# MyrtleSoftware/myrtle-vision

Measured on AMD Instinct MI355X. Metric: images/sec (train fwd+bwd) ViT-B/16 224^2 bf16, higher is better.
Workload: dtype bf16

## Files before the change

### include/myrtle_vision_hip.h

```cpp
#ifndef MYRTLE_VISION_HIP_H
#define MYRTLE_VISION_HIP_H

#include <stddef.h>
#include <stdint.h>

#ifdef __cplusplus
extern "C" {
#endif

typedef void* mv_stream_t;

enum { MV_F32 = 0, MV_BF16 = 1, MV_I8 = 2 , MV_F16 = 3  };

enum {
  MV_OK = 0,
  MV_ERR_SHAPE = -1,
  MV_ERR_ALIGN = -2,
  MV_ERR_LAUNCH = -3,
  MV_ERR_UNSUPPORTED = -4,
  MV_ERR_WORKSPACE = -5
};

enum {
  MV_EPI_NONE = 0,
  MV_EPI_GELU = 1,
  MV_EPI_RESIDUAL = 2,
  MV_EPI_DGELU = 3,
  MV_EPI_GELU_GRAD = 5,
  MV_EPI_MUL = 6,
  MV_EPI_GELU_Q8 = 7,
  MV_EPI_GELU_GRAD8 = 8,
  MV_EPI_MUL8 = 9,
  MV_EPI_SPLIT_DGELU = 10,
  MV_EPI_SPLIT_GELU = 11,
  MV_EPI_EMBED = 4
};

int mv_version(void);
const char* mv_error_string(int code);
size_t mv_gemm_tn_workspace_bytes(int M, int N, int Kc);
int mv_gemm_force_variant(int nt_variant, int tn_variant);
size_t mv_layernorm_bwd_workspace_bytes(int rows, int dim);

int mv_layernorm_fwd(const float* x, long ldx, const float* gamma, const float* beta, void* y, int y_dtype,
                     float* mean, float* rstd, int rows, int dim, float eps, mv_stream_t stream);
int mv_layernorm_fwd_split(const float* x, long ldx, const float* gamma, const float* beta, void* y_split, int nseg, float* mean,
                           float* rstd, int rows, int dim, float eps, mv_stream_t stream);
int mv_layernorm_bwd(const void* dy, int dy_dtype, const float* x, long ldx, const float* gamma,
                     const float* mean, const float* rstd, const float* dx_add, float* dx, long lddx,
                     float* dgamma, float* dbeta, int accumulate, float* workspace, size_t workspace_bytes,
                     int rows, int dim, void* dx_bf16, float* dx_colsum, mv_stream_t stream);
int mv_layernorm_bwd_split(const void* dy, int dy_dtype, const float* x, long ldx, const float* gamma, const float* mean,
                           const float* rstd, const float* dx_add, float* dx, long lddx, float* dgamma, float* dbeta, int accumulate,
                           float* workspace, size_t workspace_bytes, int rows, int dim, void* dx_split, int nseg, float* dx_colsum,
                           mv_stream_t stream);

int mv_gemm_nt_bf16(const void* A, int lda, const void* B, int ldb, void* C, int ldc, int c_dtype, int M, int N,
                    int K, const float* bias, int epilogue, const void* aux, int ld_aux, int aux_i, void* out2,
                    int ld_out2, mv_stream_t stream);
int mv_gemm_nt_bf16_scaled(const void* A, int lda, const void* B, int ldb, void* C, int ldc, int c_dtype, int M, int N,
                           int K, float alpha, const float* bias, int epilogue, const void* aux, int ld_aux, int aux_i,
                           void* out2, int ld_out2, mv_stream_t stream);
int mv_gemm_tn_bf16(const void* A, int lda, const void* B, int ldb, float* C, int ldc, int M, int N, int Kc,
                    int accumulate, float* colsum, float* workspace, size_t workspace_bytes, mv_stream_t stream);

int mv_gemm_f32(const float* A, long sa_m, long sa_k, long sa_b1, long sa_b2, const float* B, long sb_k, long sb_n,
                long sb_b1, long sb_b2, float* C, long sc_m, long sc_n, long sc_b1, long sc_b2, int M, int N, int K,
                int nb1, int nb2, float alpha, int accumulate, const float* bias, int epilogue, const float* aux,
                long ld_aux, int aux_i, float* out2, long ld_out2, mv_stream_t stream);
int mv_sum_slabs(const float* slabs, long stride, int S, float* out, long n, int accumulate, mv_stream_t stream);
int mv_sum_slabs_add(const float* slabs, long stride, int S, const float* add, float* out, long n, mv_stream_t stream);
int mv_gemm_f32_force_fma(int on);

int mv_attention_fwd(const void* qkv, void* out, float* lse, int B, int N, int H, float scale, mv_stream_t stream);
int mv_attention_bwd(const void* qkv, const void* out, const void* dout, const float* lse, void* dqkv, float* colsum,
                     int B, int N, int H, float scale, mv_stream_t stream);
int mv_attention_fwd_f16(const void* qkv16, float* out, float* lse, int B, int N, int H, float scale, mv_stream_t stream);
int mv_attention_bwd_prep_f16(const float* dout, const float* out, void* dout16, float* delta, float* gscale, int B, int N, int H,
                              mv_stream_t stream);
int mv_attention_bwd_f16(const void* qkv16, const void* dout16, const float* delta, const float* lse, const float* gscale,
                         void* dqkv, int nseg, float* colsum, int B, int N, int H, float scale, mv_stream_t stream);
int mv_attention_bwd_force(int variant);
int mv_attention_fwd_force(int variant);
int mv_attention_fwd_f32(const float* qkv, float* out, int B, int N, int H, float scale, mv_stream_t stream);

int mv_softmax_fwd(const float* x, float* y, long rows, int cols, float scale, mv_stream_t stream);
int mv_softmax_bwd(const float* y, const float* dy, float* dx, long rows, int cols, float scale, mv_stream_t stream);

int mv_patchify(const float* img, void* out, int out_dtype, int B, int C, int H, int W, int p, mv_stream_t stream);
int mv_embed_cls(const float* cls, const float* pos, float* x, int B, int T, int D, mv_stream_t stream);
int mv_embed_bwd(const float* dx, float* dpos, float* dcls, int accumulate, int B, int T, int D, mv_stream_t stream);
int mv_embed_bwd_gather(const float* dx, void* dy, int dy_dtype, float* dpos, float* dcls, int B, int T, int D,
                        mv_stream_t stream);
int mv_gather_patch_rows(const float* src, void* dst, int dst_dtype, int B, int T, int D, mv_stream_t stream);

int mv_cast(const void* src, int src_dtype, void* dst, int dst_dtype, long n, mv_stream_t stream);
int mv_split3_bf16(const float* x, long ldx, void* out, long ldo, long seg, long rows, int cols, int role,
                   mv_stream_t stream);
size_t mv_split3_ex_workspace_bytes(long rows, int cols);
int mv_split3_bf16_ex(const float* x, long ldx, const float* h, long ldh, int op, void* out, long rows, int cols,
                      float* colsum, float* workspace, size_t workspace_bytes, mv_stream_t stream);
int mv_gemm_nt_bf16_ksplit(const void* A, int lda, const void* B, int ldb, float* slabs, int M, int N, int K, int splits,
                           const float* bias, mv_stream_t stream);
int mv_gemm_tn_bf16_x6(const void* A6, const void* B6, float* C, int ldc, int M, int N, int rows, float* workspace,
                       size_t workspace_bytes, mv_stream_t stream);
int mv_split2_bf16(const float* x, long ldx, void* out, long ldo, long seg, long rows, int cols, int role,
                   mv_stream_t stream);
int mv_split2_bf16_ex(const float* x, long ldx, const float* h, long ldh, int op, void* out, long rows, int cols,
                      float* colsum, float* workspace, size_t workspace_bytes, mv_stream_t stream);
int mv_weight_split(const float* w, void* fwd, void* dx, int R, int C, int nseg, mv_stream_t stream);
int mv_split_f8c(const float* x, long ldx, void* out, long ldo_bytes, long rows, int cols, int role, int exp_hi, mv_stream_t stream);
int mv_gemm_nt_f8c(const void* A, long lda_bytes, const void* B, long ldb_bytes, void* C, int ldc, int c_dtype, int M, int N, int K,
                   int scale_exp, const float* bias, int epilogue, const void* aux, int ld_aux, mv_stream_t stream);
int mv_gemm_tn_bf16_x3(const void* A3, const void* B3, float* C, int ldc, int M, int N, int rows, float* workspace,
                       size_t workspace_bytes, mv_stream_t stream);
int mv_weight_prep(const float* w, void* w_bf16, int ldw, void* wt_bf16, int ldt, int R, int C, mv_stream_t stream);
typedef struct mv_weight_prep_item {
  const float* w;
  void* w_bf16;
  void* wt_bf16;
  int ldw, ldt, R, C;
  int tiles_x, first_block;
} mv_weight_prep_item;
int mv_weight_prep_batch(const mv_weight_prep_item* items_device, int count, int total_blocks, mv_stream_t stream);
int mv_colsum(const void* x, int x_dtype, long ld, float* out, int accumulate, long rows, int cols, float* workspace,
              size_t workspace_bytes, mv_stream_t stream);
int mv_gelu_fwd(const void* x, void* y, int dtype, long n, mv_stream_t stream);
int mv_gelu_bwd(const void* x, const void* dy, void* dx, int dtype, long n, mv_stream_t stream);
int mv_add_f32(const float* a, const float* b, float* out, long n, mv_stream_t stream);

int mv_quant_float(const float* x, float* y, long n, int exp_bits, int man_bits, mv_stream_t stream);
int mv_quant_fixed(const float* x, float* y, long n, int wl, int fl, int clamp, int symmetric, mv_stream_t stream);
int mv_quant_affine(const float* x, float* y, long n, float scale, int zero_point, int qmin, int qmax,
                    mv_stream_t stream);
int mv_quant_affine_codes(const void* x, int x_dtype, void* codes, long rows, int cols, int ld, float scale, int zero_point,
                          int qmin, int qmax, int pre_op, mv_stream_t stream);
int mv_quant_float_f16(const float* x, void* y, long n, mv_stream_t stream);
int mv_gemm_nt_f16(const void* A, int lda, const void* B, int ldb, void* C, int ldc, int M, int N, int K, const float* bias,
                   int epilogue, const void* aux, int ld_aux, void* out2, int ld_out2, mv_stream_t stream);
int mv_quant_affine_i8(const void* x, int x_dtype, void* codes, long rows, int cols, int ld, float scale, int zero_point,
                       int pre_op, mv_stream_t stream);
int mv_gemm_nt_i8(const void* A, int lda, const void* B, int ldb, void* C, int ldc, int c_dtype, int M, int N, int K,
                  float alpha, const float* bias, const int* icorr, int epilogue, const void* aux, int ld_aux,
                  float q_scale, int q_zero_point, mv_stream_t stream);
int mv_attention_fwd_f32_lse(const float* qkv, float* out, float* lse, int B, int N, int H, float scale, mv_stream_t stream);
// ... 51 lines not shown
```

### myrtle-vision_amd/csrc/gemm_bf16.hip

```cpp
#include "mv_common.h"

#include <atomic>
#include <type_traits>

namespace {

constexpr int BM = 128, BN = 128, BK = 64;
constexpr int STAGE_BYTES = (BM + BN) * BK * 2;
constexpr int SMEM_BYTES = 2 * STAGE_BYTES;

__device__ __forceinline__ int sw128(int row, int ch) { return row * 128 + ((ch ^ (((row >> 1) & 3) << 1)) << 4); }
__device__ __forceinline__ int sw256(int row, int ch) {
  return row * 256 + ((ch ^ (((row & 3) << 2) | ((row >> 2) & 3))) << 4);
}

__device__ __forceinline__ int xcd_remap(int bid, int nwg) {
  const int q = nwg >> 3, r = nwg & 7, xcd = bid & 7, idx = bid >> 3;
  return (xcd < r ? xcd * (q + 1) : r * (q + 1) + (xcd - r) * q) + idx;
}

struct EpiArgs {
  float alpha;
  const float* bias;
  const void* aux;
  int ld_aux;
  int aux_i;
  void* out2;
  int ld_out2;
  const int* icorr;
  float q_inv, q_zp;
  int ks_tiles, ks_len;
  long ks_slab;
  int band;
  int f8_tiles16, f8_scale;
};

__device__ __forceinline__ void st16(void* p, u32x4 v) { *reinterpret_cast<u32x4*>(p) = v; }

template <typename CT>
__device__ __forceinline__ void store4(CT* p, const float v[4], bool vec, int nvalid) {
  if (vec) {
    if constexpr (sizeof(CT) == 4) {
      *reinterpret_cast<float4*>(p) = make_float4(v[0], v[1], v[2], v[3]);
    } else {
      typedef CT ct4 __attribute__((ext_vector_type(4)));
      const ct4 o = {(CT)v[0], (CT)v[1], (CT)v[2], (CT)v[3]};
      *reinterpret_cast<ct4*>(p) = o;
    }
  } else {
#pragma unroll
    for (int r = 0; r < 4; ++r)
      if (r < nvalid) p[r] = (CT)v[r];
  }
}

__device__ __forceinline__ void nt_colsum_flush(float (&cs)[4][4], float* __restrict__ partial, int ld, int row_block, int nb,
                                                int N, int lane) {
#pragma unroll
  for (int j = 0; j < 4; ++j)
#pragma unroll
    for (int r = 0; r < 4; ++r) {
      float v = cs[j][r];
      v += __shfl_xor(v, 1, 64);
      v += __shfl_xor(v, 2, 64);
      v += __shfl_xor(v, 4, 64);
      v += __shfl_xor(v, 8, 64);
      cs[j][r] = v;
    }
  if ((lane & 15) == 0) {
#pragma unroll
    for (int j = 0; j < 4; ++j)
#pragma unroll
      for (int r = 0; r < 4; ++r) {
        const int n = nb + j * 16 + r;
        if (n < N) partial[(long)row_block * ld + n] = cs[j][r];
      }
  }
}

__device__ __forceinline__ float erf_fast(float u, float& e) { return mv_erf_fast(u, e); }
__device__ __forceinline__ float gelu_fast(float x) {
  float e;
  return 0.5f * x * (1.0f + erf_fast(x * 0.70710678118654752440f, e));
}
__device__ __forceinline__ void gelu_both_fast(float x, float& gl, float& dg) {
  float e;
  const float cdf = 0.5f * (1.0f + erf_fast(x * 0.70710678118654752440f, e));
  gl = x * cdf;
  dg = fmaf(x * 0.39894228040143267794f, e, cdf);
}
constexpr bool epi_is_gelu(int e) { return e == MV_EPI_GELU || e == MV_EPI_GELU_GRAD || e == MV_EPI_GELU_GRAD8; }
constexpr bool epi_is_dgelu(int e) { return e == MV_EPI_DGELU || e == MV_EPI_MUL || e == MV_EPI_MUL8; }
constexpr bool epi_is_gelugrad(int e) { return e == MV_EPI_GELU_GRAD || e == MV_EPI_GELU_GRAD8; }
constexpr bool epi_is_split(int e) { return e == MV_EPI_SPLIT_DGELU || e == MV_EPI_SPLIT_GELU; }
__device__ __forceinline__ void store_pieces4(bf16_t* o, const float (&v)[4], int nseg, long seg) {
  bf16x4 p[3];
#pragma unroll
  for (int e = 0; e < 4; ++e) {
    const bf16_t p0 = (bf16_t)v[e];
    const float r1 = v[e] - (float)p0;
    const bf16_t p1 = (bf16_t)r1;
    p[0][e] = p0;
    p[1][e] = p1;
    p[2][e] = (bf16_t)(r1 - (float)p1);
  }
  *reinterpret_cast<bf16x4*>(o) = p[0];
  *reinterpret_cast<bf16x4*>(o + seg) = p[0];
  *reinterpret_cast<bf16x4*>(o + 2 * seg) = p[1];
  if (nseg == 6) {
    *reinterpret_cast<bf16x4*>(o + 3 * seg) = p[0];
    *reinterpret_cast<bf16x4*>(o + 4 * seg) = p[1];
    *reinterpret_cast<bf16x4*>(o + 5 * seg) = p[2];
  }
}
constexpr float GQ_STEP = 0.005f, GQ_INV = 200.0f, GQ_ZERO = 26.0f;
__device__ __forceinline__ unsigned gq_code(float g) {
  return (unsigned)__builtin_amdgcn_fmed3f(fmaf(g, GQ_INV, GQ_ZERO + 0.5f), 0.f, 255.f);
}
__device__ __forceinline__ unsigned gq_pack4(const float (&g)[4]) {
  return gq_code(g[0]) | (gq_code(g[1]) << 8) | (gq_code(g[2]) << 16) | (gq_code(g[3]) << 24);
}
__device__ __forceinline__ float gq_value(float code) { return (code - GQ_ZERO) * GQ_STEP; }
__device__ __forceinline__ float gq_decode(unsigned w, int k) { return gq_value((float)((w >> (8 * k)) & 255u)); }
__device__ __forceinline__ float dgelu_fast(float x) {
  float e;
  const float cdf = 0.5f * (1.0f + erf_fast(x * 0.70710678118654752440f, e));
  return fmaf(x * 0.39894228040143267794f, e, cdf);
}

template <typename CT = bf16_t>
__device__ __forceinline__ u32x4 pair_swap_bf16(const float (&va)[4], const float (&vb)[4]) {
  typedef CT ct4 __attribute__((ext_vector_type(4)));
  const ct4 pa = {(CT)va[0], (CT)va[1], (CT)va[2], (CT)va[3]};
  const ct4 pb = {(CT)vb[0], (CT)vb[1], (CT)vb[2], (CT)vb[3]};
  typedef unsigned u32x2_t __attribute__((ext_vector_type(2)));
  const u32x2_t a = __builtin_bit_cast(u32x2_t, pa), b = __builtin_bit_cast(u32x2_t, pb);
  const u32x2_t r0 = __builtin_amdgcn_permlane16_swap(a[0], b[0], false, false);
  const u32x2_t r1 = __builtin_amdgcn_permlane16_swap(a[1], b[1], false, false);
  return (u32x4){r0[0], r1[0], r0[1], r1[1]};
}

template <int EPI>
struct EpiPre {
  float4 ax[EPI == MV_EPI_RESIDUAL ? 4 : 1][EPI == MV_EPI_RESIDUAL ? 4 : 1];
  u32x4 xq[EPI == MV_EPI_MUL8 ? 4 : 1];
};
template <int EPI>
__device__ __forceinline__ void nt_epi_prefetch(EpiPre<EPI>& P, int m0, int n0, int wm, int wn, int lane, const EpiArgs& ep) {
  const int mb = m0 + wm * 64 + (lane & 15), nb = n0 + wn * 64 + 4 * (lane >> 4);
  if constexpr (EPI == MV_EPI_RESIDUAL) {
#pragma unroll
    for (int i = 0; i < 4; ++i)
#pragma unroll
      for (int j = 0; j < 4; ++j)
        P.ax[i][j] = *reinterpret_cast<const float4*>(reinterpret_cast<const float*>(ep.aux) + (long)(mb + i * 16) * ep.ld_aux + nb + j * 16);
  } else if constexpr (EPI == MV_EPI_MUL8) {
    const unsigned char* a8 = reinterpret_cast<const unsigned char*>(ep.aux);
#pragma unroll
    for (int i = 0; i < 4; ++i)
      P.xq[i] = *reinterpret_cast<const u32x4*>(a8 + (long)(mb + i * 16) * ep.ld_aux + n0 + wn * 64 + 16 * (lane >> 4));
  }
}
template <int EPI>
__device__ __forceinline__ bool nt_epi_prefetch_ok(int M, int N, int m0, int n0, int ldc, const EpiArgs& ep) {
  const bool interior = (m0 + BM <= M) && (n0 + BN <= N) && ((ldc & 3) == 0) && ((ep.ld_aux & 3) == 0) &&
                        ((ep.ld_out2 & 3) == 0) && ((reinterpret_cast<uintptr_t>(ep.bias) & 15) == 0);
  if constexpr (EPI == MV_EPI_MUL8)
    return interior && (ep.ld_aux & 15) == 0 && (reinterpret_cast<uintptr_t>(ep.aux) & 15) == 0;
  return interior && EPI == MV_EPI_RESIDUAL;
}

template <int EPI, typename CT, bool PRE = false>
__device__ __forceinline__ void nt_epilogue(f32x4 (&acc)[4][4], CT* __restrict__ C, int ldc, int M, int N, int m0, int n0,
                                            int wm, int wn, int lane, const EpiArgs& ep, const float* bias_lds = nullptr,
                                            const EpiPre<EPI>& pre = EpiPre<EPI>{}) {
  const bool interior = (m0 + BM <= M) && (n0 + BN <= N) && ((ldc & 3) == 0) && ((ep.ld_aux & 3) == 0) &&
                        ((ep.ld_out2 & 3) == 0) && ((reinterpret_cast<uintptr_t>(ep.bias) & 15) == 0);
  if (interior) {
    const int mb = m0 + wm * 64 + (lane & 15), nb = n0 + wn * 64 + 4 * (lane >> 4);
    float4 bv[4];
#pragma unroll
    for (int j = 0; j < 4; ++j)
      bv[j] = bias_lds ? *reinterpret_cast<const float4*>(bias_lds + wn * 64 + 4 * (lane >> 4) + j * 16)
              : (!epi_is_dgelu(EPI) && ep.bias) ? *reinterpret_cast<const float4*>(ep.bias + nb + j * 16)
                                                : make_float4(0.f, 0.f, 0.f, 0.f);
    long crow[4];
    int prow[4];
#pragma unroll
    for (int i = 0; i < 4; ++i) {
      const int m = mb + i * 16;
      crow[i] = m;
      prow[i] = 0;
      if constexpr (EPI == MV_EPI_EMBED) {
        const int img = m / ep.aux_i;
        prow[i] = 1 + (m - img * ep.aux_i);
        crow[i] = (long)img * (ep.aux_i + 1) + prow[i];
      }
    }
    if constexpr (EPI == MV_EPI_GELU_Q8) {
      const bool wide = (ldc & 15) == 0 && (reinterpret_cast<uintptr_t>(C) & 15) == 0;
#pragma unroll
      for (int i = 0; i < 4; ++i) {
        unsigned w[4];
#pragma unroll
        for (int j = 0; j < 4; ++j) {
          const float v0 = fmaf(acc[i][j][0], ep.alpha, bv[j].x), v1 = fmaf(acc[i][j][1], ep.alpha, bv[j].y);
          const float v2 = fmaf(acc[i][j][2], ep.alpha, bv[j].z), v3 = fmaf(acc[i][j][3], ep.alpha, bv[j].w);
          w[j] = affine_i8_pack4<1>(v0, v1, v2, v3, ep.q_inv, ep.q_zp);
        }
        char* crow8 = reinterpret_cast<char*>(C) + (long)(mb + i * 16) * ldc;
        if (wide) {
          typedef unsigned u32x2_t __attribute__((ext_vector_type(2)));
          const u32x2_t s01 = __builtin_amdgcn_permlane16_swap(w[0], w[1], false, false);
          const u32x2_t s23 = __builtin_amdgcn_permlane16_swap(w[2], w[3], false, false);
          const u32x2_t t02 = __builtin_amdgcn_permlane32_swap(s01[0], s23[0], false, false);
          const u32x2_t t13 = __builtin_amdgcn_permlane32_swap(s01[1], s23[1], false, false);
          st16(crow8 + n0 + wn * 64 + 16 * (lane >> 4), (u32x4){t02[0], t13[0], t02[1], t13[1]});
        } else {
#pragma unroll
          for (int j = 0; j < 4; ++j) *reinterpret_cast<unsigned*>(crow8 + nb + j * 16) = w[j];
        }
      }
      return;
    }
    float4 ax[4][4];
    if constexpr (EPI == MV_EPI_RESIDUAL || EPI == MV_EPI_EMBED || EPI == MV_EPI_SPLIT_DGELU) {
#pragma unroll
      for (int i = 0; i < 4; ++i)
#pragma unroll
        for (int j = 0; j < 4; ++j) {
          if constexpr (EPI == MV_EPI_RESIDUAL && PRE) {
            ax[i][j] = pre.ax[i][j];
            continue;
          }
          const long arow = (EPI == MV_EPI_EMBED) ? prow[i] : (mb + i * 16);
          ax[i][j] = *reinterpret_cast<const float4*>(reinterpret_cast<const float*>(ep.aux) + arow * ep.ld_aux + nb + j * 16);
        }
    }
    bf16x4 hx[4][4];
    unsigned hq[4][4];
    if constexpr (EPI == MV_EPI_MUL8) {
      const unsigned char* a8 = reinterpret_cast<const unsigned char*>(ep.aux);
      if ((ep.ld_aux & 15) == 0 && (reinterpret_cast<uintptr_t>(a8) & 15) == 0) {
        typedef unsigned u32x2_t __attribute__((ext_vector_type(2)));
        u32x4 x[4];
#pragma unroll
        for (int i = 0; i < 4; ++i)
          x[i] = PRE ? pre.xq[i]
                     : *reinterpret_cast<const u32x4*>(a8 + (long)(mb + i * 16) * ep.ld_aux + n0 + wn * 64 + 16 * (lane >> 4));
#pragma unroll
        for (int i = 0; i < 4; ++i) {
          const u32x2_t s01 = __builtin_amdgcn_permlane16_swap(x[i][0], x[i][1], false, false);
          const u32x2_t s23 = __builtin_amdgcn_permlane16_swap(x[i][2], x[i][3], false, false);
          const u32x2_t t02 = __builtin_amdgcn_permlane32_swap(s01[0], s23[0], false, false);
          const u32x2_t t13 = __builtin_amdgcn_permlane32_swap(s01[1], s23[1], false, false);
// ... 42 lines not shown
                    gelu_both_fast(v[q][r], gl, dg);
                    hpre[q][r] = dg;
                    v[q][r] = gl;
                  } else {
                    hpre[q][r] = v[q][r];
                    v[q][r] = gelu_fast(v[q][r]);
                  }
                }
              } else if constexpr (epi_is_dgelu(EPI)) {
#pragma unroll
                for (int r = 0; r < 4; ++r)
                  v[q][r] *= (EPI == MV_EPI_MUL8) ? gq_decode(hq[i][j], r)
                             : (EPI == MV_EPI_MUL) ? (float)hx[i][j][r] : dgelu_fast((float)hx[i][j][r]);
                cs[j][0] += v[q][0]; cs[j][1] += v[q][1]; cs[j][2] += v[q][2]; cs[j][3] += v[q][3];
              }
            }
            if constexpr (EPI == MV_EPI_GELU_GRAD8) {
              gw[2 * jp] = gq_pack4(hpre[0]);
              gw[2 * jp + 1] = gq_pack4(hpre[1]);
            } else if constexpr (epi_is_gelu(EPI)) {
              if (ep.out2)
                st16(reinterpret_cast<bf16_t*>(ep.out2) + (long)(mb + i * 16) * ep.ld_out2 + nw + 32 * jp,
                     pair_swap_bf16(hpre[0], hpre[1]));
            }
            st16(C + crow[i] * ldc + nw + 32 * jp, pair_swap_bf16<CT>(v[0], v[1]));
          }
          if constexpr (EPI == MV_EPI_GELU_GRAD8) {
            if (ep.out2) {
              typedef unsigned u32x2_t __attribute__((ext_vector_type(2)));
              const u32x2_t s01 = __builtin_amdgcn_permlane16_swap(gw[0], gw[1], false, false);
              const u32x2_t s23 = __builtin_amdgcn_permlane16_swap(gw[2], gw[3], false, false);
              const u32x2_t t02 = __builtin_amdgcn_permlane32_swap(s01[0], s23[0], false, false);
              const u32x2_t t13 = __builtin_amdgcn_permlane32_swap(s01[1], s23[1], false, false);
              st16(reinterpret_cast<unsigned char*>(ep.out2) + (long)(mb + i * 16) * ep.ld_out2 + n0 + wn * 64 + 16 * (lane >> 4),
                   (u32x4){t02[0], t13[0], t02[1], t13[1]});
            }
          }
        }
        if constexpr (epi_is_dgelu(EPI)) {
          if (ep.out2) nt_colsum_flush(cs, reinterpret_cast<float*>(ep.out2), ep.ld_out2, (m0 + wm * 64) >> 6, nb, N, lane);
        }
        return;
      }
    }
#pragma unroll
    for (int i = 0; i < 4; ++i)
#pragma unroll
      for (int j = 0; j < 4; ++j) {
        float v[4] = {fmaf(acc[i][j][0], ep.alpha, bv[j].x), fmaf(acc[i][j][1], ep.alpha, bv[j].y),
                      fmaf(acc[i][j][2], ep.alpha, bv[j].z), fmaf(acc[i][j][3], ep.alpha, bv[j].w)};
        const int n = nb + j * 16;
        if constexpr (epi_is_gelu(EPI)) {
          float o2[4] = {v[0], v[1], v[2], v[3]};
#pragma unroll
          for (int r = 0; r < 4; ++r) {
            if constexpr (epi_is_gelugrad(EPI)) gelu_both_fast(o2[r], v[r], o2[r]);
            else v[r] = gelu_fast(v[r]);
          }
          if constexpr (EPI == MV_EPI_GELU_GRAD8) {
            if (ep.out2)
              *reinterpret_cast<unsigned*>(reinterpret_cast<unsigned char*>(ep.out2) + (long)(mb + i * 16) * ep.ld_out2 + n) =
                  gq_pack4(o2);
          } else {
            if (ep.out2) store4(reinterpret_cast<bf16_t*>(ep.out2) + (long)(mb + i * 16) * ep.ld_out2 + n, o2, true, 4);
          }
        } else if constexpr (EPI == MV_EPI_RESIDUAL || EPI == MV_EPI_EMBED) {
          v[0] += ax[i][j].x; v[1] += ax[i][j].y; v[2] += ax[i][j].z; v[3] += ax[i][j].w;
        } else if constexpr (EPI == MV_EPI_SPLIT_DGELU) {
          v[0] *= dgelu_f(ax[i][j].x); v[1] *= dgelu_f(ax[i][j].y); v[2] *= dgelu_f(ax[i][j].z); v[3] *= dgelu_f(ax[i][j].w);
          cs[j][0] += v[0]; cs[j][1] += v[1]; cs[j][2] += v[2]; cs[j][3] += v[3];
        } else if constexpr (EPI == MV_EPI_SPLIT_GELU) {
          st16(reinterpret_cast<float*>(ep.out2) + (long)(mb + i * 16) * ep.ld_out2 + n,
               __builtin_bit_cast(u32x4, (f32x4){v[0], v[1], v[2], v[3]}));
          v[0] = gelu_f(v[0]); v[1] = gelu_f(v[1]); v[2] = gelu_f(v[2]); v[3] = gelu_f(v[3]);
        } else if constexpr (epi_is_dgelu(EPI)) {
#pragma unroll
          for (int r = 0; r < 4; ++r)
            v[r] *= (EPI == MV_EPI_MUL8) ? gq_decode(hq[i][j], r)
                    : (EPI == MV_EPI_MUL) ? (float)hx[i][j][r] : dgelu_fast((float)hx[i][j][r]);
          cs[j][0] += v[0]; cs[j][1] += v[1]; cs[j][2] += v[2]; cs[j][3] += v[3];
        }
        if constexpr (epi_is_split(EPI))
          store_pieces4(reinterpret_cast<bf16_t*>(C) + crow[i] * ldc + n, v, ep.aux_i, N);
        else if constexpr (sizeof(CT) == 4)
          st16(C + crow[i] * ldc + n, __builtin_bit_cast(u32x4, (f32x4){v[0], v[1], v[2], v[3]}));
        else
          store4(C + crow[i] * ldc + n, v, true, 4);
      }
    if constexpr (epi_is_dgelu(EPI) || EPI == MV_EPI_SPLIT_DGELU) {
      if (ep.out2) nt_colsum_flush(cs, reinterpret_cast<float*>(ep.out2), ep.ld_out2, (m0 + wm * 64) >> 6, nb, N, lane);
    }
    return;
  }
  const bool ldc_vec = (ldc & 3) == 0;
  float cs[4][4];
#pragma unroll
  for (int j = 0; j < 4; ++j)
#pragma unroll
    for (int r = 0; r < 4; ++r) cs[j][r] = 0.f;
#pragma unroll
  for (int i = 0; i < 4; ++i) {
    const int m = m0 + wm * 64 + i * 16 + (lane & 15);
    if (m >= M) continue;
    long crow = m;
    int patch = 0;
    if constexpr (EPI == MV_EPI_EMBED) {
      const int img = m / ep.aux_i;
      patch = m - img * ep.aux_i;
      crow = (long)img * (ep.aux_i + 1) + 1 + patch;
    }
#pragma unroll
    for (int j = 0; j < 4; ++j) {
      const int n = n0 + wn * 64 + j * 16 + 4 * (lane >> 4);
      if (n >= N) continue;
      const int nvalid = (N - n) >= 4 ? 4 : (N - n);
      const bool vec = ldc_vec && nvalid == 4;
      float v[4] = {acc[i][j][0] * ep.alpha, acc[i][j][1] * ep.alpha, acc[i][j][2] * ep.alpha, acc[i][j][3] * ep.alpha};
      if (ep.bias) {
#pragma unroll
        for (int r = 0; r < 4; ++r)
          if (r < nvalid) v[r] += ep.bias[n + r];
      }
      if constexpr (epi_is_gelu(EPI)) {
        float o2[4] = {v[0], v[1], v[2], v[3]};
#pragma unroll
        for (int r = 0; r < 4; ++r) {
          if constexpr (epi_is_gelugrad(EPI)) gelu_both_fast(o2[r], v[r], o2[r]);
          else v[r] = gelu_fast(v[r]);
        }
        if constexpr (EPI == MV_EPI_GELU_GRAD8) {
          if (ep.out2) {
            unsigned char* o8 = reinterpret_cast<unsigned char*>(ep.out2) + (long)m * ep.ld_out2 + n;
#pragma unroll
            for (int r = 0; r < 4; ++r)
              if (r < nvalid) o8[r] = (unsigned char)gq_code(o2[r]);
          }
        } else {
          if (ep.out2) store4(reinterpret_cast<bf16_t*>(ep.out2) + (long)m * ep.ld_out2 + n, o2, vec && (ep.ld_out2 & 3) == 0, nvalid);
        }
      } else if constexpr (EPI == MV_EPI_RESIDUAL) {
        const float* ax = reinterpret_cast<const float*>(ep.aux) + (long)m * ep.ld_aux + n;
#pragma unroll
        for (int r = 0; r < 4; ++r)
          if (r < nvalid) v[r] += ax[r];
      } else if constexpr (EPI == MV_EPI_MUL8) {
        const unsigned char* ax = reinterpret_cast<const unsigned char*>(ep.aux) + (long)m * ep.ld_aux + n;
#pragma unroll
        for (int r = 0; r < 4; ++r)
          if (r < nvalid) {
            v[r] *= gq_value((float)ax[r]);
            cs[j][r] += v[r];
          }
      } else if constexpr (epi_is_dgelu(EPI)) {
        const bf16_t* ax = reinterpret_cast<const bf16_t*>(ep.aux) + (long)m * ep.ld_aux + n;
#pragma unroll
        for (int r = 0; r < 4; ++r)
          if (r < nvalid) {
            v[r] *= (EPI == MV_EPI_MUL) ? (float)ax[r] : dgelu_fast((float)ax[r]);
            cs[j][r] += v[r];
          }
      } else if constexpr (EPI == MV_EPI_EMBED) {
        const float* ax = reinterpret_cast<const float*>(ep.aux) + (long)(1 + patch) * ep.ld_aux + n;
#pragma unroll
        for (int r = 0; r < 4; ++r)
          if (r < nvalid) v[r] += ax[r];
      }
// ... 232 lines not shown
#pragma unroll
    for (int j = 0; j < 4; ++j) acc[i][j] = (f32x4){0.f, 0.f, 0.f, 0.f};

  const int nk = K / BKR;
  const int frag_off = (lane & 15) * 64 + (((lane >> 4) ^ (((lane >> 3) & 1) << 1)) << 4);
#pragma unroll
  for (int s = 0; s < S - 1; ++s)
    if (s < nk) RING_ISSUE(s, s)
  int slot = 0, fill = S - 1;
#define RING_SYNC(kt_)                                                                                     \
  {                                                                                                        \
    if ((kt_) + S - 2 < nk) {                                                                              \
      asm volatile("s_waitcnt vmcnt(%0)" ::"n"(4 * (S - 2)) : "memory");             \
    } else {                                                                                               \
      asm volatile("s_waitcnt vmcnt(0)" ::: "memory");                                                     \
    }                                                                                                      \
    __builtin_amdgcn_s_barrier();      \
    asm volatile("" ::: "memory");                                                                         \
  }
#define RING_REFILL(kt_)                                                                                   \
  {                                                                                                        \
    if ((kt_) + S - 1 < nk) RING_ISSUE(fill, (kt_) + S - 1)       \
  }
#define RING_READ()                                                                                        \
  {                                                                                                        \
    const char* sa_ = smem + slot * RSTAGE_BYTES + wm * 128 * 64 + frag_off;                               \
    const char* sb_ = smem + slot * RSTAGE_BYTES + BM2 * BKR * 2 + wn * 64 * 64 + frag_off;                \
    _Pragma("unroll") for (int j = 0; j < 4; ++j) bfr[j] = *reinterpret_cast<const bf16x8*>(sb_ + j * 1024); \
    _Pragma("unroll") for (int i = 0; i < 8; ++i) af[i] = *reinterpret_cast<const bf16x8*>(sa_ + i * 1024);  \
  }
#define RING_MFMA()                                                                                        \
  {                                                                                                        \
    _Pragma("unroll") for (int i = 0; i < 8; ++i)                                                          \
      _Pragma("unroll") for (int j = 0; j < 4; ++j)                                                        \
        acc[i][j] = __builtin_amdgcn_mfma_f32_16x16x32_bf16(bfr[j], af[i], acc[i][j], 0, 0, 0);            \
  }
#define RING_ADVANCE()                                                                                     \
  {                                                                                                        \
    asm volatile("s_waitcnt lgkmcnt(0)" ::: "memory");  \
    slot = (slot + 1 == S) ? 0 : slot + 1;                                                                 \
    fill = (fill + 1 == S) ? 0 : fill + 1;                                                                 \
  }
  bf16x8 af[8], bfr[4];
  if (__builtin_amdgcn_readfirstlane(wave) < 4) {
    for (int kt = 0; kt < nk; ++kt) {
      RING_SYNC(kt)
      RING_REFILL(kt)
      RING_READ()
      RING_MFMA()
      RING_ADVANCE()
    }
  } else {
    for (int kt = 0; kt < nk; ++kt) {
      RING_SYNC(kt)
      if (kt > 0) RING_MFMA()
      RING_REFILL(kt)
      RING_READ()
      RING_ADVANCE()
    }
    if (nk > 0) RING_MFMA()
  }
#undef RING_REFILL
#undef RING_SYNC
#undef RING_READ
#undef RING_MFMA
#undef RING_ADVANCE
#undef RING_ISSUE
#pragma unroll
  for (int h = 0; h < 2; ++h)
    nt_epilogue<EPI, CT>(*reinterpret_cast<f32x4(*)[4][4]>(&acc[4 * h]), C, ldc, M, N, m0 + 128 * wm, n0 + 128 * (wn >> 1), h,
                         wn & 1, lane, ep);
}

constexpr int P8_SLOT = 128 * 64 * 2;
constexpr int P8_SMEM = 8 * P8_SLOT;
constexpr int P8_BQ0 = 0, P8_AQ0 = 1, P8_BQ1 = 2, P8_AQ1 = 3;

typedef __attribute__((ext_vector_type(4))) int i32x4;

constexpr int NT_BF16 = 0, NT_I8 = 1, NT_F16 = 2, NT_F8C = 3;
typedef __attribute__((ext_vector_type(8))) int i32x8;
typedef __attribute__((ext_vector_type(8))) _Float16 f16x8;

template <int EPI, typename CT, int OPK = NT_BF16, bool KSPLIT = false>
__global__ __launch_bounds__(512, 2) void gemm_nt_8phase_kernel(const bf16_t* __restrict__ A, int lda,
                                                                const bf16_t* __restrict__ B, int ldb, CT* __restrict__ C,
                                                                int ldc, int M, int N, int K, int tiles_n, EpiArgs ep,
                                                                int full_tiles, int item0) {
  extern __shared__ __attribute__((aligned(16))) char smem[];
  constexpr bool I8 = OPK == NT_I8;
  const int tid = threadIdx.x, lane = tid & 63, wave = tid >> 6;
  const int wm = wave >> 2, wn = wave & 3;
  const int bid = blockIdx.x + item0;
  const int nk = K >> 6;
  int t, half = -1;
  if (bid < full_tiles) {
    t = xcd_remap(bid, full_tiles);
    if (!KSPLIT && ep.band > 0) {
      const int rows = full_tiles / tiles_n, per_band = rows * ep.band;
      if (t < rows * tiles_n) {
        const int b = t / per_band, r = t - b * per_band, rm = r / ep.band;
        t = rm * tiles_n + b * ep.band + (r - rm * ep.band);
      }
    }
  } else {
    const int idx = bid - full_tiles;
    t = full_tiles + (idx >> 1);
    half = idx & 1;
  }
  const bool is_half_rt = half >= 0;
  if constexpr (KSPLIT) {
    const int ks = t / ep.ks_tiles;
    t -= ks * ep.ks_tiles;
    A += (long)ks * ep.ks_len;
    B += (long)ks * ep.ks_len;
    C += (long)ks * ep.ks_slab;
    if (ks) ep.bias = nullptr;
  }
  auto body = [&](auto half_tag) {
  constexpr bool is_half = decltype(half_tag)::value;
  const int m0 = (t / tiles_n) * BM2 + (is_half ? 128 * half : 0), n0 = (t % tiles_n) * BN2;

  unsigned ps[4][2];
#pragma unroll
  for (int i = 0; i < 2; ++i) {
    const int rloc = 16 * wave + 8 * i + (lane >> 3);
    const int ch = (lane & 7) ^ (((rloc >> 1) & 3) << 1);
    const int ra = m0 + (is_half ? 64 : 128) * (wave >> 2) + 16 * (wave & 3) + 8 * i + (lane >> 3);
    const int rb = n0 + 64 * (wave >> 1) + 16 * (wave & 1) + 8 * i + (lane >> 3);
    const int ra0 = ra < M ? ra : M - 1, ra1 = ra + 64 < M ? ra + 64 : M - 1;
    const int rb0 = rb < N ? rb : N - 1, rb1 = rb + 32 < N ? rb + 32 : N - 1;
    ps[P8_AQ0][i] = (unsigned)ra0 * (unsigned)lda + ch * 8;
    ps[P8_AQ1][i] = (unsigned)ra1 * (unsigned)lda + ch * 8;
    ps[P8_BQ0][i] = (unsigned)rb0 * (unsigned)ldb + ch * 8;
    ps[P8_BQ1][i] = (unsigned)rb1 * (unsigned)ldb + ch * 8;
  }
  char* const wave_lds = smem + __builtin_amdgcn_readfirstlane(wave) * 2048;
  const __amdgpu_buffer_rsrc_t rsA = __builtin_amdgcn_make_buffer_rsrc(const_cast<bf16_t*>(A), (short)0, (int)((unsigned)M * (unsigned)lda * 2u), 0x00020000);
  const __amdgpu_buffer_rsrc_t rsB = __builtin_amdgcn_make_buffer_rsrc(const_cast<bf16_t*>(B), (short)0, (int)((unsigned)N * (unsigned)ldb * 2u), 0x00020000);
#define P8_STAGE(buf_, slot_, kt_)                                                      \
  {                                                                                     \
    char* l_ = wave_lds + ((buf_) * 4 + (slot_)) * P8_SLOT;                             \
    const int so_ = (kt_) * 128;                                                        \
    if ((slot_) == P8_AQ0 || (slot_) == P8_AQ1) {                                       \
      __builtin_amdgcn_raw_ptr_buffer_load_lds(rsA, LDS_PTR(void, l_), 16, (int)(ps[slot_][0] * 2u), so_, 0, 0);        \
      __builtin_amdgcn_raw_ptr_buffer_load_lds(rsA, LDS_PTR(void, l_ + 1024), 16, (int)(ps[slot_][1] * 2u), so_, 0, 0); \
    } else {                                                                            \
      __builtin_amdgcn_raw_ptr_buffer_load_lds(rsB, LDS_PTR(void, l_), 16, (int)(ps[slot_][0] * 2u), so_, 0, 0);        \
      __builtin_amdgcn_raw_ptr_buffer_load_lds(rsB, LDS_PTR(void, l_ + 1024), 16, (int)(ps[slot_][1] * 2u), so_, 0, 0); \
    }                                                                                   \
  }

  f32x4 acc[8][4];
#pragma unroll
  for (int i = 0; i < 8; ++i)
#pragma unroll
    for (int j = 0; j < 4; ++j) acc[i][j] = (f32x4){0.f, 0.f, 0.f, 0.f};

  const int fr = (((lane & 15) >> 1) & 3) << 1;
  const int rf0 = (lane & 15) * 128 + (((lane >> 4) ^ fr) << 4);
  const int rf1 = (lane & 15) * 128 + (((4 + (lane >> 4)) ^ fr) << 4);
  const char* const a_rd = smem + 64 * wm * 128;
  const char* const b_rd = smem + 32 * wn * 128;
  bf16x8 af[4][2], bf0[2][2], bf1[2][2];
  [[maybe_unused]] i32x8 af_8[4], bf0_8[2], bf1_8[2];
#define P8_PAIR(p0_, p1_)                                                                                    \
  __builtin_shufflevector(*reinterpret_cast<const i32x4*>(p0_), *reinterpret_cast<const i32x4*>(p1_), 0, 1, 2, 3, 4, 5, 6, 7)
#define P8_READ_A(buf_, slot_)                                                                               \
  {                                                                                                          \
    const char* s_ = a_rd + ((buf_) * 4 + (slot_)) * P8_SLOT;                                                \
    _Pragma("unroll") for (int i = 0; i < 4; ++i) {                                                          \
      if constexpr (OPK == NT_F8C) {                                                                         \
        af_8[i] = P8_PAIR(s_ + i * 2048 + rf0, s_ + i * 2048 + rf1);                                         \
      } else {                                                                                               \
        af[i][0] = *reinterpret_cast<const bf16x8*>(s_ + i * 2048 + rf0);                                    \
        af[i][1] = *reinterpret_cast<const bf16x8*>(s_ + i * 2048 + rf1);                                    \
      }                                                                                                      \
    }                                                                                                        \
  }
#define P8_READ_B(dst_, buf_, slot_)                                                                         \
  {                                                                                                          \
    const char* s_ = b_rd + ((buf_) * 4 + (slot_)) * P8_SLOT;                                                \
    _Pragma("unroll") for (int j = 0; j < 2; ++j) {                                                          \
      if constexpr (OPK == NT_F8C) {                                                                         \
        dst_##_8[j] = P8_PAIR(s_ + j * 2048 + rf0, s_ + j * 2048 + rf1);                                     \
      } else {                                                                                               \
        dst_[j][0] = *reinterpret_cast<const bf16x8*>(s_ + j * 2048 + rf0);                                  \
        dst_[j][1] = *reinterpret_cast<const bf16x8*>(s_ + j * 2048 + rf1);                                  \
      }                                                                                                      \
    }                                                                                                        \
  }
#define P8_MFMA(mb_, nb_, bfx_, M8_)                                                                         \
  {                                                                                                          \
// ... 55 lines not shown
    if (lazy) { W1_ }                                                                                        \
    P8_BAR()                                                                                                 \
    P8_LGKM0()                                                                                               \
    P8_MFMA(0, 0, bf0, M8_)                                                                                       \
    P8_BAR()                                                                                                 \
                                                                                              \
    P8_READ_B(bf1, d_, P8_BQ1)                                                                               \
    __builtin_amdgcn_sched_barrier(0);                                                                       \
    if (ST_) P8_STAGE(next_buf_, P8_BQ0, next_kt_)                                                           \
    if (lazy) { W2_ }                                                                                        \
    P8_BAR()                                                                                                 \
    P8_LGKM0()                                                                                               \
    P8_MFMA(0, 2, bf1, M8_)                                                                                       \
    P8_BAR()                                                                                                 \
                                                                                              \
    if (!is_half) P8_READ_A(d_, P8_AQ1)                                                                      \
    __builtin_amdgcn_sched_barrier(0);                                                                       \
    if (ST_) P8_STAGE(next_buf_, P8_AQ0, next_kt_)                                                           \
    P8_BAR()                                                                                                 \
    P8_LGKM0()                                                                                               \
    if (!is_half) P8_MFMA(4, 2, bf1, M8_)                                                                         \
    P8_BAR()                                                                                                 \
                                                                                              \
    if (ST_) P8_STAGE(next_buf_, P8_BQ1, next_kt_)                                                           \
    if (lazy) { W4_ } else { H4_ }                                                                           \
    P8_BAR()                                                                                                 \
    if (!is_half) P8_MFMA(4, 0, bf0, M8_)                                                                         \
    P8_BAR()                                                                                                 \
  }

  constexpr bool lazy = !is_half;
  P8_STAGE(0, P8_BQ0, 0) P8_STAGE(0, P8_AQ0, 0) P8_STAGE(0, P8_BQ1, 0) if (!is_half) P8_STAGE(0, P8_AQ1, 0)
  P8_STAGE(1, P8_BQ0, 1) P8_STAGE(1, P8_AQ0, 1) P8_STAGE(1, P8_BQ1, 1)
  if (lazy) { P8_WAIT(10) } else { P8_WAIT(6) }
  P8_BAR()
  if (__builtin_amdgcn_readfirstlane(wave) >= 4) P8_BAR()
  int kt = 0;
  [[maybe_unused]] const int f8_sc = (ep.f8_scale & 255) * 0x01010101;
  if constexpr (OPK == NT_F8C) {
    for (; kt < ep.f8_tiles16; kt += 2) {
      P8_KTILE(0, 1, 1, kt + 1, 0, kt + 2, P8_WAIT(10), P8_WAIT(10), P8_WAIT(10), P8_WAIT(6), 1, 0)
      P8_KTILE(1, 1, 0, kt + 2, 1, kt + 3, P8_WAIT(10), P8_WAIT(10), P8_WAIT(10), P8_WAIT(6), 1, 0)
    }
    for (; kt < nk - 2; kt += 2) {
      P8_KTILE(0, 1, 1, kt + 1, 0, kt + 2, P8_WAIT(10), P8_WAIT(10), P8_WAIT(10), P8_WAIT(6), 1, 1)
      P8_KTILE(1, 1, 0, kt + 2, 1, kt + 3, P8_WAIT(10), P8_WAIT(10), P8_WAIT(10), P8_WAIT(6), 1, 1)
    }
    P8_KTILE(0, 0, 1, kt + 1, 0, 0, P8_WAIT(10), P8_WAIT(8), P8_WAIT(4), P8_WAIT(0), 1, 1)
    P8_KTILE(1, 0, 0, 0, 0, 0, P8_WAIT(2), P8_WAIT(0), , , 0, 1)
  } else {
  for (; kt < nk - 2; kt += 2) {
    P8_KTILE(0, 1, 1, kt + 1, 0, kt + 2, P8_WAIT(10), P8_WAIT(10), P8_WAIT(10), P8_WAIT(6), 1, 0)
    P8_KTILE(1, 1, 0, kt + 2, 1, kt + 3, P8_WAIT(10), P8_WAIT(10), P8_WAIT(10), P8_WAIT(6), 1, 0)
  }
  P8_KTILE(0, 0, 1, kt + 1, 0, 0, P8_WAIT(10), P8_WAIT(8), P8_WAIT(4), P8_WAIT(0), 1, 0)
  P8_KTILE(1, 0, 0, 0, 0, 0, P8_WAIT(2), P8_WAIT(0), , , 0, 0)
  }
  if (__builtin_amdgcn_readfirstlane(wave) < 4) P8_BAR()
#undef P8_WAIT
#undef P8_KTILE
#undef P8_LGKM0
#undef P8_BAR
#undef P8_MFMA
#undef P8_READ_A
#undef P8_PAIR
#undef P8_READ_B
#undef P8_STAGE
  if constexpr (I8) {
    const int nc = n0 + 128 * (wn >> 1) + 64 * (wn & 1) + 4 * (lane >> 4);
#pragma unroll
    for (int j = 0; j < 4; ++j) {
      int c[4] = {0, 0, 0, 0};
      if (ep.icorr) {
#pragma unroll
        for (int r = 0; r < 4; ++r) c[r] = (nc + 16 * j + r < N) ? ep.icorr[nc + 16 * j + r] : 0;
      }
#pragma unroll
      for (int i = 0; i < 8; ++i) {
        const i32x4 iv = __builtin_bit_cast(i32x4, acc[i][j]);
        acc[i][j] = (f32x4){(float)(iv[0] + c[0]), (float)(iv[1] + c[1]), (float)(iv[2] + c[2]), (float)(iv[3] + c[3])};
      }
    }
  }
  constexpr bool park = epi_is_dgelu(EPI) || EPI == MV_EPI_RESIDUAL || EPI == MV_EPI_SPLIT_DGELU;
  f32x4* const parked = reinterpret_cast<f32x4*>(smem) + wave * 16 * 64 + lane;
  if (park && !is_half) {
#pragma unroll
    for (int i = 0; i < 4; ++i)
#pragma unroll
      for (int j = 0; j < 4; ++j) parked[(i * 4 + j) * 64] = acc[4 + i][j];
  }
  constexpr bool can_pre = (EPI == MV_EPI_RESIDUAL || EPI == MV_EPI_MUL8) && !KSPLIT;
  if constexpr (can_pre) {
    if (!is_half && nt_epi_prefetch_ok<EPI>(M, N, m0 + 128 * wm, n0 + 128 * (wn >> 1), ldc, ep)) {
      EpiPre<EPI> pre0, pre1;
      nt_epi_prefetch<EPI>(pre0, m0 + 128 * wm, n0 + 128 * (wn >> 1), 0, wn & 1, lane, ep);
      nt_epi_prefetch<EPI>(pre1, m0 + 128 * wm, n0 + 128 * (wn >> 1), 1, wn & 1, lane, ep);
      nt_epilogue<EPI, CT, true>(*reinterpret_cast<f32x4(*)[4][4]>(&acc[0]), C, ldc, M, N, m0 + 128 * wm, n0 + 128 * (wn >> 1), 0,
                                 wn & 1, lane, ep, nullptr, pre0);
      f32x4 accb[4][4];
#pragma unroll
      for (int i = 0; i < 4; ++i)
#pragma unroll
        for (int j = 0; j < 4; ++j) accb[i][j] = parked[(i * 4 + j) * 64];
      nt_epilogue<EPI, CT, true>(accb, C, ldc, M, N, m0 + 128 * wm, n0 + 128 * (wn >> 1), 1, wn & 1, lane, ep, nullptr, pre1);
      return;
    }
  }
  nt_epilogue<EPI, CT>(*reinterpret_cast<f32x4(*)[4][4]>(&acc[0]), C, ldc, M, N, is_half ? m0 : m0 + 128 * wm,
                       n0 + 128 * (wn >> 1), is_half ? wm : 0, wn & 1, lane, ep);
  if (is_half) return;
  f32x4 acc2[4][4];
  if (park) {
#pragma unroll
    for (int i = 0; i < 4; ++i)
#pragma unroll
      for (int j = 0; j < 4; ++j) acc2[i][j] = parked[(i * 4 + j) * 64];
  } else {
#pragma unroll
    for (int i = 0; i < 4; ++i)
#pragma unroll
      for (int j = 0; j < 4; ++j) acc2[i][j] = acc[4 + i][j];
  }
  nt_epilogue<EPI, CT>(acc2, C, ldc, M, N, m0 + 128 * wm, n0 + 128 * (wn >> 1), 1, wn & 1, lane, ep);
  };
  if (is_half_rt) body(std::true_type{});
  else body(std::false_type{});
}

__device__ __forceinline__ void tn_store(f32x4 (&acc)[4][4], float* __restrict__ Cs, long ldc, int M, int N, int m0, int n0,
                                         int wm, int wn, int lane) {
  const bool ldc_vec = (ldc & 3) == 0;
#pragma unroll
  for (int i = 0; i < 4; ++i) {
    const int m = m0 + wm * 64 + i * 16 + (lane & 15);
    if (m >= M) continue;
#pragma unroll
    for (int j = 0; j < 4; ++j) {
      const int n = n0 + wn * 64 + j * 16 + 4 * (lane >> 4);
      if (n >= N) continue;
      const int nvalid = (N - n) >= 4 ? 4 : (N - n);
      const float v[4] = {acc[i][j][0], acc[i][j][1], acc[i][j][2], acc[i][j][3]};
      store4(Cs + (long)m * ldc + n, v, ldc_vec && nvalid == 4, nvalid);
    }
  }
}


__global__ __launch_bounds__(256, 2) void gemm_tn_kernel(const bf16_t* __restrict__ A, int lda,
                                                         const bf16_t* __restrict__ B, int ldb, float* __restrict__ C,
                                                         long ldc, long slab_stride, int M, int N, int Kc, int tiles_n,
                                                         int tiles_mn, int steps_per_split) {
  extern __shared__ __attribute__((aligned(16))) char smem[];
  const int tid = threadIdx.x, lane = tid & 63, wave = tid >> 6;
  const int wm = wave >> 1, wn = wave & 1;
  const int t_all = xcd_remap(blockIdx.x, gridDim.x);
  const int split = t_all / tiles_mn;
  const int t = t_all - split * tiles_mn;
  const int m0 = (t / tiles_n) * BM, n0 = (t % tiles_n) * BN;
  const int nk_total = (Kc + BK - 1) / BK;
  const int kt0 = split * steps_per_split;
  int nk = nk_total - kt0;
  if (nk > steps_per_split) nk = steps_per_split;
  float* Cs = C + (long)split * slab_stride;

  const int sc = tid & 15, sr = tid >> 4;
  u32x4 ra0, ra1, ra2, ra3, rb0, rb1, rb2, rb3;
  const u32x4 zero4 = {0u, 0u, 0u, 0u};
  const bool a_in = (m0 + sc * 8) < M, b_in = (n0 + sc * 8) < N;
  const bf16_t* pa = A + (a_in ? m0 + sc * 8 : 0);
  const bf16_t* pb = B + (b_in ? n0 + sc * 8 : 0);
  const int kc_last = Kc - 1;
#define TN_LOAD_TILE(kt_)                                                                 \
  {                                                                                       \
    const int kc_ = (kt0 + (kt_)) * BK + sr;                                              \
    const bool k0_ = kc_ < Kc, k1_ = kc_ + 16 < Kc, k2_ = kc_ + 32 < Kc, k3_ = kc_ + 48 < Kc; \
    const long r0_ = k0_ ? kc_ : kc_last, r1_ = k1_ ? kc_ + 16 : kc_last;                 \
    const long r2_ = k2_ ? kc_ + 32 : kc_last, r3_ = k3_ ? kc_ + 48 : kc_last;            \
    ra0 = *reinterpret_cast<const u32x4*>(pa + r0_ * lda);                                \
    ra1 = *reinterpret_cast<const u32x4*>(pa + r1_ * lda);                                \
    ra2 = *reinterpret_cast<const u32x4*>(pa + r2_ * lda);                                \
    ra3 = *reinterpret_cast<const u32x4*>(pa + r3_ * lda);                                \
    rb0 = *reinterpret_cast<const u32x4*>(pb + r0_ * ldb);                                \
    rb1 = *reinterpret_cast<const u32x4*>(pb + r1_ * ldb);                                \
    rb2 = *reinterpret_cast<const u32x4*>(pb + r2_ * ldb);                                \
    rb3 = *reinterpret_cast<const u32x4*>(pb + r3_ * ldb);                                \
    ra0 = (k0_ && a_in) ? ra0 : zero4; ra1 = (k1_ && a_in) ? ra1 : zero4;                 \
    ra2 = (k2_ && a_in) ? ra2 : zero4; ra3 = (k3_ && a_in) ? ra3 : zero4;                 \
    rb0 = (k0_ && b_in) ? rb0 : zero4; rb1 = (k1_ && b_in) ? rb1 : zero4;                 \
    rb2 = (k2_ && b_in) ? rb2 : zero4; rb3 = (k3_ && b_in) ? rb3 : zero4;                 \
  }
#define TN_STORE_TILE(stage_)                                                             \
  {                                                                                       \
    char* sa_ = smem + (stage_) * STAGE_BYTES;                                            \
    char* sb_ = sa_ + BK * BM * 2;                                                        \
    *reinterpret_cast<u32x4*>(sa_ + sw256(sr, sc)) = ra0;                                 \
    *reinterpret_cast<u32x4*>(sa_ + sw256(sr + 16, sc)) = ra1;                            \
    *reinterpret_cast<u32x4*>(sa_ + sw256(sr + 32, sc)) = ra2;                            \
    *reinterpret_cast<u32x4*>(sa_ + sw256(sr + 48, sc)) = ra3;                            \
    *reinterpret_cast<u32x4*>(sb_ + sw256(sr, sc)) = rb0;                                 \
    *reinterpret_cast<u32x4*>(sb_ + sw256(sr + 16, sc)) = rb1;                            \
    *reinterpret_cast<u32x4*>(sb_ + sw256(sr + 32, sc)) = rb2;                            \
    *reinterpret_cast<u32x4*>(sb_ + sw256(sr + 48, sc)) = rb3;                            \
  }

  f32x4 acc[4][4];
#pragma unroll
  for (int i = 0; i < 4; ++i)
#pragma unroll
    for (int j = 0; j < 4; ++j) acc[i][j] = (f32x4){0.f, 0.f, 0.f, 0.f};
// ... 332 lines not shown
    const int i = threadIdx.x;
    partial[(long)blockIdx.y * cols + cc] = (red[0][i] + red[1][i]) + (red[2][i] + red[3][i]);
  }
}

int colsum_parts(long rows) {
  long p = (rows + 255) / 256;
  if (p < 1) p = 1;
  if (p > 256) p = 256;
  return (int)p;
}

std::atomic<int> g_force_nt{getenv("MV_GEMM_TILE") ? atoi(getenv("MV_GEMM_TILE")) : 0};
std::atomic<int> g_force_tn{getenv("MV_GEMM_TN") ? atoi(getenv("MV_GEMM_TN")) : 0};

struct TnPlan {
  int tiles_m, tiles_n, splits, steps_per_split;
};

TnPlan tn_plan(int M, int N, int Kc) {
  TnPlan pl;
  pl.tiles_m = mv_cdiv(M, BM);
  pl.tiles_n = mv_cdiv(N, BN);
  const int tiles = pl.tiles_m * pl.tiles_n;
  const int nk = mv_cdiv(Kc, BK) < 1 ? 1 : mv_cdiv(Kc, BK);
  int s = mv_cdiv(512, tiles);
  const int max_s = mv_cdiv(nk, 8);
  if (s > max_s) s = max_s;
  if (s > 64) s = 64;
  if (s < 1) s = 1;
  pl.steps_per_split = mv_cdiv(nk, s);
  pl.splits = mv_cdiv(nk, pl.steps_per_split);
  return pl;
}

TnPlan tn_plan256(int M, int N, int Kc) {
  TnPlan pl;
  pl.tiles_m = mv_cdiv(M, BM2);
  pl.tiles_n = mv_cdiv(N, BN2);
  const int tiles = pl.tiles_m * pl.tiles_n;
  const int nk = Kc / BKR;
  int s = 256 / tiles;
  const int max_s = mv_cdiv(nk, 16);
  if (s > max_s) s = max_s;
  if (s < 1) s = 1;
  pl.steps_per_split = mv_cdiv(nk, s);
  pl.splits = mv_cdiv(nk, pl.steps_per_split);
  return pl;
}
bool tn_use_ring(int M, int N, int Kc) {
  const int force = g_force_tn.load(std::memory_order_relaxed);
  if (Kc <= 0 || Kc % BKR != 0 || force == 128) return false;
  if (force == 256) return true;
  if (!((long)M * N >= 256L * 256 * 4 && Kc >= 4096)) return false;
  const TnPlan pl = tn_plan256(M, N, Kc);
  return pl.tiles_m * pl.tiles_n * pl.splits >= 160;
}

template <typename K>
int set_smem(K kernel) {
  return hipFuncSetAttribute(reinterpret_cast<const void*>(kernel), hipFuncAttributeMaxDynamicSharedMemorySize,
                             SMEM_BYTES) == hipSuccess
             ? 0
             : -1;
}

constexpr int NT_CUS = 256;
inline int nt_full_tiles(int tiles) {
  const int tail = tiles % NT_CUS;
  return (tiles >= NT_CUS && tail > 0 && 2 * tail <= NT_CUS) ? tiles - tail : tiles;
}

constexpr int NT_FEATURES_DEFAULT = 2;
inline int nt_band_width(int tiles_n, int K, bool whole_tiles_only) {
  static const int forced = getenv("MV_NT_BAND") ? atoi(getenv("MV_NT_BAND")) : 0;
  if (forced > 0) return tiles_n % forced == 0 && tiles_n > forced ? forced : 0;
  (void)whole_tiles_only;
  return (tiles_n == 9 && K <= 1024) ? 3 : 0;
}

template <int EPI, typename CT>
int launch_nt(const void* A, int lda, const void* B, int ldb, void* C, int ldc, int M, int N, int K, EpiArgs ep,
              hipStream_t s) {
  const int attr = MV_ONCE_PER_DEVICE(set_smem(gemm_nt_kernel<EPI, CT>) | set_smem(gemm_nt_glds_kernel<EPI, CT>) |
                          set_smem(gemm_nt_glds_kernel<EPI, CT, false>));
  if (attr != 0) return MV_ERR_LAUNCH;
  const int tiles_m = mv_cdiv(M, BM), tiles_n = mv_cdiv(N, BN);
  const int t2m = mv_cdiv(M, BM2), t2n = mv_cdiv(N, BN2);
  int force = g_force_nt.load(std::memory_order_relaxed);
  int feat = NT_FEATURES_DEFAULT;
  if (force == 3000 || force == 3002) {
    feat = force - 3000;
    force = 0;
  } else if (force == 3100 || force == 3102) {
    feat = force - 3100;
    force = 2568;
  }
  const bool ring_ok = K > 0 && K % BKR == 0;
  const bool ring_pick = ring_ok && ((long)t2m * t2n >= 1024 || (K >= 2048 && (long)t2m * t2n >= 256));
  const bool p8_ok = K >= 128 && K % 128 == 0 && (long)M * lda < (1L << 31) && (long)N * ldb < (1L << 31);
  const long t2 = (long)t2m * t2n;
  const bool p8_halves = p8_ok && !ring_pick && t2 >= NT_CUS / 4 && t2 < NT_CUS / 2;
  const bool p8_pick = p8_ok && (ring_pick || t2 >= NT_CUS / 4);
  if (((force == 2568 || force == 25680 || force == 25681) && p8_ok) || (force == 0 && p8_pick)) {
    const int a8 = MV_ONCE_PER_DEVICE(hipFuncSetAttribute(reinterpret_cast<const void*>(gemm_nt_8phase_kernel<EPI, CT>),
                                              hipFuncAttributeMaxDynamicSharedMemorySize, P8_SMEM) == hipSuccess ? 0 : -1);
    if (a8) return MV_ERR_LAUNCH;
    const int tiles = t2m * t2n,
              full = force == 25680 ? tiles : (force == 25681 || (force == 0 && p8_halves)) ? 0 : nt_full_tiles(tiles);
    if (feat & 2) ep.band = nt_band_width(t2n, K, full == tiles);
    gemm_nt_8phase_kernel<EPI, CT><<<full + 2 * (tiles - full), 512, P8_SMEM, s>>>(
        (const bf16_t*)A, lda, (const bf16_t*)B, ldb, (CT*)C, ldc, M, N, K, t2n, ep, full, 0);
    MV_CHECK_LAUNCH();
    return MV_OK;
  }
  if ((force == 2564 && ring_ok) || (force == 0 && ring_pick)) {
    const int a4 = MV_ONCE_PER_DEVICE(hipFuncSetAttribute(reinterpret_cast<const void*>(gemm_nt_ring_kernel<EPI, CT, 4>),
                                              hipFuncAttributeMaxDynamicSharedMemorySize, 4 * RSTAGE_BYTES) == hipSuccess ? 0 : -1);
    if (a4) return MV_ERR_LAUNCH;
    gemm_nt_ring_kernel<EPI, CT, 4><<<t2m * t2n, 512, 4 * RSTAGE_BYTES, s>>>((const bf16_t*)A, lda, (const bf16_t*)B, ldb,
                                                                              (CT*)C, ldc, M, N, K, t2n, ep);
  } else if (K > 0 && K % BK == 0) {
    if ((long)M * lda < (1L << 31) && (long)N * ldb < (1L << 31))
      gemm_nt_glds_kernel<EPI, CT><<<tiles_m * tiles_n, 256, SMEM_BYTES, s>>>((const bf16_t*)A, lda, (const bf16_t*)B, ldb,
                                                                               (CT*)C, ldc, M, N, K, tiles_n, ep);
    else
      gemm_nt_glds_kernel<EPI, CT, false><<<tiles_m * tiles_n, 256, SMEM_BYTES, s>>>((const bf16_t*)A, lda, (const bf16_t*)B, ldb,
                                                                                      (CT*)C, ldc, M, N, K, tiles_n, ep);
  }
  else
    gemm_nt_kernel<EPI, CT><<<tiles_m * tiles_n, 256, SMEM_BYTES, s>>>((const bf16_t*)A, lda, (const bf16_t*)B, ldb,
                                                                        (CT*)C, ldc, M, N, K, tiles_n, ep);
  MV_CHECK_LAUNCH();
  return MV_OK;
}

}

extern "C" int mv_gemm_nt_bf16_scaled(const void* A, int lda, const void* B, int ldb, void* C, int ldc, int c_dtype, int M,
                                      int N, int K, float alpha, const float* bias, int epilogue, const void* aux, int ld_aux,
                                      int aux_i, void* out2, int ld_out2, mv_stream_t stream);

extern "C" int mv_gemm_nt_bf16(const void* A, int lda, const void* B, int ldb, void* C, int ldc, int c_dtype, int M,
                               int N, int K, const float* bias, int epilogue, const void* aux, int ld_aux, int aux_i,
                               void* out2, int ld_out2, mv_stream_t stream) {
  return mv_gemm_nt_bf16_scaled(A, lda, B, ldb, C, ldc, c_dtype, M, N, K, 1.0f, bias, epilogue, aux, ld_aux, aux_i, out2,
                                ld_out2, stream);
}

extern "C" int mv_gemm_nt_bf16_scaled(const void* A, int lda, const void* B, int ldb, void* C, int ldc, int c_dtype, int M,
                                      int N, int K, float alpha, const float* bias, int epilogue, const void* aux, int ld_aux,
                                      int aux_i, void* out2, int ld_out2, mv_stream_t stream) {
  MV_REQUIRE(M >= 0 && N >= 0 && K >= 0, MV_ERR_SHAPE);
  if (M == 0 || N == 0) return MV_OK;
  MV_REQUIRE(lda % 8 == 0 && ldb % 8 == 0 && lda >= ((K + 7) & ~7) && ldb >= ((K + 7) & ~7), MV_ERR_ALIGN);
  MV_REQUIRE(mv_aligned16(A) && mv_aligned16(B) && mv_aligned16(C), MV_ERR_ALIGN);
  hipStream_t s = (hipStream_t)stream;
  EpiArgs ep{alpha, bias, aux, ld_aux, aux_i, out2, ld_out2, nullptr, 0.f, 0.f};
  switch (epilogue) {
    case MV_EPI_NONE:
      if (c_dtype == MV_F16)
        return launch_nt<MV_EPI_NONE, _Float16>(A, lda, B, ldb, C, ldc, M, N, K, ep, s);
      return c_dtype == MV_F32 ? launch_nt<MV_EPI_NONE, float>(A, lda, B, ldb, C, ldc, M, N, K, ep, s)
                               : launch_nt<MV_EPI_NONE, bf16_t>(A, lda, B, ldb, C, ldc, M, N, K, ep, s);
    case MV_EPI_GELU:
      MV_REQUIRE(c_dtype == MV_BF16, MV_ERR_UNSUPPORTED);
      return launch_nt<MV_EPI_GELU, bf16_t>(A, lda, B, ldb, C, ldc, M, N, K, ep, s);
    case MV_EPI_RESIDUAL:
      MV_REQUIRE(c_dtype == MV_F32 && aux, MV_ERR_UNSUPPORTED);
      return launch_nt<MV_EPI_RESIDUAL, float>(A, lda, B, ldb, C, ldc, M, N, K, ep, s);
    case MV_EPI_DGELU:
      MV_REQUIRE(c_dtype == MV_BF16 && aux, MV_ERR_UNSUPPORTED);
      return launch_nt<MV_EPI_DGELU, bf16_t>(A, lda, B, ldb, C, ldc, M, N, K, ep, s);
    case MV_EPI_GELU_GRAD:
      MV_REQUIRE(c_dtype == MV_BF16, MV_ERR_UNSUPPORTED);
      return launch_nt<MV_EPI_GELU_GRAD, bf16_t>(A, lda, B, ldb, C, ldc, M, N, K, ep, s);
    case MV_EPI_MUL:
      MV_REQUIRE(c_dtype == MV_BF16 && aux, MV_ERR_UNSUPPORTED);
      return launch_nt<MV_EPI_MUL, bf16_t>(A, lda, B, ldb, C, ldc, M, N, K, ep, s);
    case MV_EPI_GELU_GRAD8:
      MV_REQUIRE(c_dtype == MV_BF16, MV_ERR_UNSUPPORTED);
      return launch_nt<MV_EPI_GELU_GRAD8, bf16_t>(A, lda, B, ldb, C, ldc, M, N, K, ep, s);
    case MV_EPI_MUL8:
      MV_REQUIRE(c_dtype == MV_BF16 && aux, MV_ERR_UNSUPPORTED);
      return launch_nt<MV_EPI_MUL8, bf16_t>(A, lda, B, ldb, C, ldc, M, N, K, ep, s);
    case MV_EPI_EMBED:
      MV_REQUIRE(c_dtype == MV_F32 && aux && aux_i > 0, MV_ERR_UNSUPPORTED);
      return launch_nt<MV_EPI_EMBED, float>(A, lda, B, ldb, C, ldc, M, N, K, ep, s);
    case MV_EPI_SPLIT_DGELU:
    case MV_EPI_SPLIT_GELU: {
      MV_REQUIRE(c_dtype == MV_BF16 && (aux_i == 3 || aux_i == 6) && M % 256 == 0 && N % 256 == 0 && K % 128 == 0 && K >= 128,
                 MV_ERR_UNSUPPORTED);
      MV_REQUIRE(ldc >= aux_i * N && ldc % 4 == 0, MV_ERR_ALIGN);
      if (epilogue == MV_EPI_SPLIT_DGELU) {
        MV_REQUIRE(aux && ld_aux % 4 == 0 && mv_aligned16(aux) && !bias, MV_ERR_ALIGN);
        return launch_nt<MV_EPI_SPLIT_DGELU, bf16_t>(A, lda, B, ldb, C, ldc, M, N, K, ep, s);
      }
      MV_REQUIRE(out2 && ld_out2 % 4 == 0 && mv_aligned16(out2), MV_ERR_ALIGN);
      return launch_nt<MV_EPI_SPLIT_GELU, bf16_t>(A, lda, B, ldb, C, ldc, M, N, K, ep, s);
    }
    default:
      return MV_ERR_UNSUPPORTED;
  }
}

extern "C" int mv_gemm_nt_bf16_ksplit(const void* A, int lda, const void* B, int ldb, float* slabs, int M, int N, int K,
                                      int splits, const float* bias, mv_stream_t stream) {
  MV_REQUIRE(M > 0 && N > 0 && K > 0 && splits >= 1, MV_ERR_SHAPE);
  MV_REQUIRE(K % (128 * splits) == 0 && N % 4 == 0, MV_ERR_UNSUPPORTED);
  MV_REQUIRE(lda % 8 == 0 && ldb % 8 == 0 && lda >= K && ldb >= K, MV_ERR_ALIGN);
  MV_REQUIRE(mv_aligned16(A) && mv_aligned16(B) && mv_aligned16(slabs), MV_ERR_ALIGN);
  MV_REQUIRE((long)M * lda < (1L << 31) && (long)N * ldb < (1L << 31), MV_ERR_UNSUPPORTED);
  const int a8 = MV_ONCE_PER_DEVICE(hipFuncSetAttribute(reinterpret_cast<const void*>(gemm_nt_8phase_kernel<MV_EPI_NONE, float, NT_BF16, true>),
                                            hipFuncAttributeMaxDynamicSharedMemorySize, P8_SMEM) == hipSuccess ? 0 : -1);
  if (a8) return MV_ERR_LAUNCH;
  const int t2m = mv_cdiv(M, BM2), t2n = mv_cdiv(N, BN2);
  const int tiles = t2m * t2n, items = tiles * splits, full = nt_full_tiles(items);
  EpiArgs ep{1.0f, bias, nullptr, 0, 0, nullptr, 0, nullptr, 0.f, 0.f, tiles, K / splits, (long)M * N};
  gemm_nt_8phase_kernel<MV_EPI_NONE, float, NT_BF16, true><<<full + 2 * (items - full), 512, P8_SMEM, (hipStream_t)stream>>>(
      (const bf16_t*)A, lda, (const bf16_t*)B, ldb, slabs, N, M, N, K / splits, t2n, ep, full, 0);
  MV_CHECK_LAUNCH();
  return MV_OK;
}

namespace {
template <int NSEG>
int launch_tn_segments(const void* A, const void* B, float* C, int ldc, int M, int N, int rows, float* workspace,
                       size_t workspace_bytes, hipStream_t s) {
  MV_REQUIRE(M > 0 && N > 0 && rows > 0, MV_ERR_SHAPE);
  MV_REQUIRE(M % 8 == 0 && N % 8 == 0 && rows % BKR == 0, MV_ERR_UNSUPPORTED);
  MV_REQUIRE((long)rows * NSEG * M * 2 < (1L << 32) && (long)rows * NSEG * N * 2 < (1L << 32), MV_ERR_UNSUPPORTED);
  MV_REQUIRE(mv_aligned16(A) && mv_aligned16(B) && mv_aligned16(C) && mv_aligned16(workspace), MV_ERR_ALIGN);
  const int Kc = NSEG * rows;
  MV_REQUIRE(workspace_bytes >= mv_gemm_tn_workspace_bytes(M, N, Kc), MV_ERR_WORKSPACE);
  const TnPlan pl = tn_plan256(M, N, Kc);
  const int tiles_mn = pl.tiles_m * pl.tiles_n;
  const bool direct = pl.splits == 1;
  const long slab_stride = (long)M * N;
  const int a4 = MV_ONCE_PER_DEVICE(hipFuncSetAttribute(reinterpret_cast<const void*>(gemm_tn_ring_kernel<4, true>),
                                            hipFuncAttributeMaxDynamicSharedMemorySize, 4 * RSTAGE_BYTES) == hipSuccess ? 0 : -1);
  if (a4) return MV_ERR_LAUNCH;
  TnSeg seg;
  seg.tiles = rows / BKR;
  const int pa[6] = {0, 0, 1, 0, 1, 2}, pb[6] = {0, 1, 0, 2, 1, 0}, block[3] = {0, 2, 5};
  for (int i = 0; i < 6; ++i) {
    const int j = i < NSEG ? i : NSEG - 1;
    seg.a[i] = block[pa[j]] * M;
    seg.b[i] = block[pb[j]] * N;
  }
  gemm_tn_ring_kernel<4, true><<<tiles_mn * pl.splits, 512, 4 * RSTAGE_BYTES, s>>>(
      (const bf16_t*)A, NSEG * M, (const bf16_t*)B, NSEG * N, direct ? C : workspace, direct ? (long)ldc : (long)N,
      direct ? 0 : slab_stride, M, N, Kc, pl.tiles_n, tiles_mn, pl.steps_per_split, seg);
  MV_CHECK_LAUNCH();
  if (!direct) {
    int grid = mv_cdiv(slab_stride, 256);
    if (grid > 2048) grid = 2048;
    splitk_reduce_kernel<<<grid, 256, 0, s>>>(workspace, slab_stride, pl.splits, C, ldc, M, N, 0);
    MV_CHECK_LAUNCH();
  }
  return MV_OK;
}
}

extern "C" int mv_gemm_tn_bf16_x6(const void* A6, const void* B6, float* C, int ldc, int M, int N, int rows, float* workspace,
                                  size_t workspace_bytes, mv_stream_t stream) {
  return launch_tn_segments<6>(A6, B6, C, ldc, M, N, rows, workspace, workspace_bytes, (hipStream_t)stream);
}

extern "C" int mv_gemm_tn_bf16_x3(const void* A3, const void* B3, float* C, int ldc, int M, int N, int rows, float* workspace,
                                  size_t workspace_bytes, mv_stream_t stream) {
  return launch_tn_segments<3>(A3, B3, C, ldc, M, N, rows, workspace, workspace_bytes, (hipStream_t)stream);
}

namespace {
template <int EPI, typename CT>
int launch_nt_i8(const void* A, int lda, const void* B, int ldb, void* C, int ldc, int M, int N, int K, EpiArgs ep,
                 hipStream_t s) {
  const int a8 = MV_ONCE_PER_DEVICE(hipFuncSetAttribute(reinterpret_cast<const void*>(gemm_nt_8phase_kernel<EPI, CT, NT_I8>),
                                            hipFuncAttributeMaxDynamicSharedMemorySize, P8_SMEM) == hipSuccess ? 0 : -1);
  if (a8) return MV_ERR_LAUNCH;
  const int t2m = mv_cdiv(M, BM2), t2n = mv_cdiv(N, BN2);
  const int tiles = t2m * t2n, full = nt_full_tiles(tiles);
  gemm_nt_8phase_kernel<EPI, CT, NT_I8><<<full + 2 * (tiles - full), 512, P8_SMEM, s>>>(
      (const bf16_t*)A, lda / 2, (const bf16_t*)B, ldb / 2, (CT*)C, ldc, M, N, K / 2, t2n, ep, full, 0);
  MV_CHECK_LAUNCH();
  return MV_OK;
}
}
// ... 212 lines not shown
```

### myrtle-vision_amd/csrc/layernorm.hip

```cpp
#include "mv_common.h"

namespace {

template <int VPL, typename YT, int NSEG = 0>
__global__ __launch_bounds__(256) void ln_fwd_kernel(const float* __restrict__ x, long ldx,
                                                     const float* __restrict__ gamma,
                                                     const float* __restrict__ beta, YT* __restrict__ y,
                                                     float* __restrict__ mean, float* __restrict__ rstd, int rows,
                                                     int dim, float eps, float q_inv = 0.f, float q_zp = 0.f) {
  const int lane = threadIdx.x & 63;
  const int wave = threadIdx.x >> 6;
  const int nvec = dim >> 2;
  const float inv_dim = 1.0f / (float)dim;
  for (long row = (long)blockIdx.x * 4 + wave; row < rows; row += (long)gridDim.x * 4) {
    const float4* xr = reinterpret_cast<const float4*>(x + row * ldx);
    float4 v[VPL];
    float s = 0.f;
#pragma unroll
    for (int i = 0; i < VPL; ++i) {
      const int c = lane + 64 * i;
      v[i] = (c < nvec) ? xr[c] : make_float4(0.f, 0.f, 0.f, 0.f);
      s += (v[i].x + v[i].y) + (v[i].z + v[i].w);
    }
    const float mu = wave_sum(s) * inv_dim;
    float q = 0.f;
#pragma unroll
    for (int i = 0; i < VPL; ++i) {
      const int c = lane + 64 * i;
      if (c < nvec) {
        const float a = v[i].x - mu, b = v[i].y - mu, cc = v[i].z - mu, d = v[i].w - mu;
        q += (a * a + b * b) + (cc * cc + d * d);
      }
    }
    const float rs = rsqrtf(wave_sum(q) * inv_dim + eps);
    if (lane == 0 && mean) {
      mean[row] = mu;
      rstd[row] = rs;
    }
    YT* yr = y + row * (long)dim * (NSEG ? NSEG : 1);
#pragma unroll
    for (int i = 0; i < VPL; ++i) {
      const int c = lane + 64 * i;
      if (c < nvec) {
        const float4 g = reinterpret_cast<const float4*>(gamma)[c];
        const float4 b = reinterpret_cast<const float4*>(beta)[c];
        const float o0 = (v[i].x - mu) * rs * g.x + b.x, o1 = (v[i].y - mu) * rs * g.y + b.y;
        const float o2 = (v[i].z - mu) * rs * g.z + b.z, o3 = (v[i].w - mu) * rs * g.w + b.w;
        if constexpr (NSEG != 0) {
          const float o[4] = {o0, o1, o2, o3};
          bf16x4 p[3];
#pragma unroll
          for (int e = 0; e < 4; ++e) {
            const bf16_t p0 = (bf16_t)o[e];
            const float r1 = o[e] - (float)p0;
            const bf16_t p1 = (bf16_t)r1;
            p[0][e] = p0;
            p[1][e] = p1;
            p[2][e] = (bf16_t)(r1 - (float)p1);
          }
          constexpr int order[6] = {0, 0, 1, 0, 1, 2};
#pragma unroll
          for (int sgm = 0; sgm < NSEG; ++sgm) reinterpret_cast<bf16x4*>(yr + (long)sgm * dim)[c] = p[order[sgm]];
        } else if constexpr (sizeof(YT) == 1) {
          reinterpret_cast<unsigned*>(yr)[c] = affine_i8_pack4<0>(o0, o1, o2, o3, q_inv, q_zp);
        } else if constexpr (sizeof(YT) == 4) {
          reinterpret_cast<float4*>(yr)[c] = make_float4(o0, o1, o2, o3);
        } else {
          bf16x4 o = {(bf16_t)o0, (bf16_t)o1, (bf16_t)o2, (bf16_t)o3};
          reinterpret_cast<bf16x4*>(yr)[c] = o;
        }
      }
    }
  }
}

template <int VPL, typename DT>
__global__ __launch_bounds__(256) void ln_bwd_kernel(const DT* __restrict__ dy, const float* __restrict__ x, long ldx,
                                                     const float* __restrict__ gamma, const float* __restrict__ mean,
                                                     const float* __restrict__ rstd, const float* dx_add, float* dx,
                                                     long lddx, float* __restrict__ partial, int rows, int dim,
                                                     bf16_t* __restrict__ dx16, int want_colsum, int dx16_nseg = 0) {
  __shared__ float red[4][VPL * 64 * 4 * 2];
  const int lane = threadIdx.x & 63;
  const int wave = threadIdx.x >> 6;
  const int nvec = dim >> 2;
  const float inv_dim = 1.0f / (float)dim;
  float4 g4[VPL], dg[VPL], db[VPL], dc[VPL];
#pragma unroll
  for (int i = 0; i < VPL; ++i) {
    const int c = lane + 64 * i;
    g4[i] = (c < nvec) ? reinterpret_cast<const float4*>(gamma)[c] : make_float4(0.f, 0.f, 0.f, 0.f);
    dg[i] = make_float4(0.f, 0.f, 0.f, 0.f);
    db[i] = make_float4(0.f, 0.f, 0.f, 0.f);
    dc[i] = make_float4(0.f, 0.f, 0.f, 0.f);
  }
  for (long row = (long)blockIdx.x * 4 + wave; row < rows; row += (long)gridDim.x * 4) {
    const float4* xr = reinterpret_cast<const float4*>(x + row * ldx);
    const DT* dyr = dy + row * (long)dim;
    const float mu = mean[row], rs = rstd[row];
    float4 xh[VPL], gg[VPL];
    float s1 = 0.f, s2 = 0.f;
#pragma unroll
    for (int i = 0; i < VPL; ++i) {
      const int c = lane + 64 * i;
      float4 d = make_float4(0.f, 0.f, 0.f, 0.f), xv = make_float4(mu, mu, mu, mu);
      if (c < nvec) {
        xv = xr[c];
        if constexpr (sizeof(DT) == 4) {
          d = reinterpret_cast<const float4*>(dyr)[c];
        } else {
          const bf16x4 t = reinterpret_cast<const bf16x4*>(dyr)[c];
          d = make_float4((float)t[0], (float)t[1], (float)t[2], (float)t[3]);
        }
      }
      xh[i] = make_float4((xv.x - mu) * rs, (xv.y - mu) * rs, (xv.z - mu) * rs, (xv.w - mu) * rs);
      gg[i] = make_float4(d.x * g4[i].x, d.y * g4[i].y, d.z * g4[i].z, d.w * g4[i].w);
      s1 += (gg[i].x + gg[i].y) + (gg[i].z + gg[i].w);
      s2 += (gg[i].x * xh[i].x + gg[i].y * xh[i].y) + (gg[i].z * xh[i].z + gg[i].w * xh[i].w);
      dg[i].x += d.x * xh[i].x; dg[i].y += d.y * xh[i].y; dg[i].z += d.z * xh[i].z; dg[i].w += d.w * xh[i].w;
      db[i].x += d.x; db[i].y += d.y; db[i].z += d.z; db[i].w += d.w;
    }
    const float c1 = wave_sum(s1) * inv_dim;
    const float c2 = wave_sum(s2) * inv_dim;
    float4* dxr = reinterpret_cast<float4*>(dx + row * lddx);
    const float4* addr = dx_add ? reinterpret_cast<const float4*>(dx_add + row * lddx) : nullptr;
#pragma unroll
    for (int i = 0; i < VPL; ++i) {
      const int c = lane + 64 * i;
      if (c < nvec) {
        float4 o = make_float4(rs * (gg[i].x - c1 - xh[i].x * c2), rs * (gg[i].y - c1 - xh[i].y * c2),
                               rs * (gg[i].z - c1 - xh[i].z * c2), rs * (gg[i].w - c1 - xh[i].w * c2));
        if (addr) {
          const float4 a = addr[c];
          o.x += a.x; o.y += a.y; o.z += a.z; o.w += a.w;
        }
        dxr[c] = o;
        if (dx16 && dx16_nseg == 0) {
          bf16x4 o16 = {(bf16_t)o.x, (bf16_t)o.y, (bf16_t)o.z, (bf16_t)o.w};
          reinterpret_cast<bf16x4*>(dx16 + row * (long)dim)[c] = o16;
        } else if (dx16) {
          const float ov[4] = {o.x, o.y, o.z, o.w};
          bf16x4 p[3];
#pragma unroll
          for (int e = 0; e < 4; ++e) {
            const bf16_t p0 = (bf16_t)ov[e];
            const float r1 = ov[e] - (float)p0;
            const bf16_t p1 = (bf16_t)r1;
            p[0][e] = p0;
            p[1][e] = p1;
            p[2][e] = (bf16_t)(r1 - (float)p1);
          }
          bf16x4* pr = reinterpret_cast<bf16x4*>(dx16 + row * (long)dim * dx16_nseg) + c;
          const int nv = dim >> 2;
          pr[0] = p[0]; pr[nv] = p[0]; pr[2 * nv] = p[1];
          if (dx16_nseg == 6) { pr[3 * nv] = p[0]; pr[4 * nv] = p[1]; pr[5 * nv] = p[2]; }
// ... 210 lines not shown
```

### myrtle-vision_amd/myrtle_vision/hip/functional.py

```python
import functools
import weakref

import torch
from torch.autograd import Function

from . import ops
from .ops import (EPI_DGELU, EPI_EMBED, EPI_GELU, EPI_GELU_GRAD, EPI_GELU_GRAD8, EPI_MUL, EPI_MUL8, EPI_NONE,
                  EPI_RESIDUAL)


GELU_GRAD_BITS = 8


def _c(t):
    return t if t.is_contiguous() else t.contiguous()


def _scoped(backward):
    @functools.wraps(backward)
    def run(ctx, *args, **kwargs):
        with ops.split_scope(), ops.segments(getattr(ctx, "mv_segments", 6)):
            return backward(ctx, *args, **kwargs)
    return run


def _fwd(forward):
    @functools.wraps(forward)
    def run(ctx, *args, **kwargs):
        prec = args[-1] if args and isinstance(args[-1], str) else None
        ctx.mv_segments = ops.prec_segments(prec) if prec is not None else getattr(ops._seg_tls, "n", 6)
        with ops.segments(ctx.mv_segments):
            return forward(ctx, *args, **kwargs)
    return run


class _LayerNorm(Function):

    @staticmethod
    @_fwd
    def forward(ctx, x, gamma, beta, out_dtype, eps):
        ops.require_cuda(x, gamma, beta)
        x = _c(x.float())
        dim = x.shape[-1]
        rows = x.numel() // dim
        y, mean, rstd = ops.layernorm_fwd(x, dim, rows, dim, gamma, beta, out_dtype, eps)
        ctx.save_for_backward(x, gamma, mean, rstd)
        ctx.beta = beta
        return y.view(x.shape)

    @staticmethod
    @_scoped
    def backward(ctx, dy):
        x, gamma, mean, rstd = ctx.saved_tensors
        dim = x.shape[-1]
        rows = x.numel() // dim
        dy = _c(dy)
        dx = torch.empty_like(x)
        dg, db = ops.layernorm_bwd(dy, x, dim, gamma, mean, rstd, None, dx, dim, rows, dim, beta=ctx.beta)
        return dx, dg, db, None, None


def layer_norm(x, gamma, beta, out_dtype=torch.float32, eps=1e-5):
    return _LayerNorm.apply(x, gamma, beta, out_dtype, eps)


class _Linear(Function):

    @staticmethod
    @_fwd
    def forward(ctx, x, weight, bias, out_dtype):
        ops.require_cuda(x, weight, bias)
        K = x.shape[-1]
        N = weight.shape[0]
        x2 = _c(x).view(-1, K)
        M = x2.shape[0]
        if x2.dtype == torch.bfloat16 and K % 8 != 0:
            raise RuntimeError(f"bf16 Linear needs in_features % 8 == 0 (got {K}); use precision='fp32'")
        out = torch.empty(M, N, dtype=out_dtype, device=x.device)
        ops.linear_fwd(x2, M, K, weight, bias, out, N)
        ctx.save_for_backward(x2, weight)
        ctx.has_bias = bias is not None
        ctx.bias = bias
        ctx.in_shape = x.shape
        return out.view(*x.shape[:-1], N)

    @staticmethod
    @_scoped
    def backward(ctx, dy):
        x2, weight = ctx.saved_tensors
        M, K = x2.shape
        N = weight.shape[0]
        dy2 = _c(dy).view(M, N)
        if dy2.dtype != x2.dtype:
            dy2 = ops.cast(dy2, x2.dtype)
# ... 276 lines not shown
        adt = ops.act_dtype(prec)
        B, C, H, W = img.shape
        npatch = (H // patch) * (W // patch)
        T, D, pd = npatch + 1, weight.shape[0], weight.shape[1]
        if adt == torch.bfloat16 and pd % 8 != 0:
            raise RuntimeError(f"bf16 patch embedding needs patch_dim % 8 == 0 (got {pd}); use precision='fp32'")
        patches = ops.patchify(img, patch, adt)
        x = torch.empty(B, T, D, dtype=torch.float32, device=img.device)
        pos2 = _c(pos.detach().float()).view(T, D)
        ops.linear_fwd(patches, B * npatch, pd, weight, bias, x, D, epi=EPI_EMBED, aux=pos2, ld_aux=D, aux_i=npatch)
        ops.embed_cls(_c(cls_token.detach()).view(D), pos2, x, B, T, D)
        ctx.save_for_backward(patches)
        ctx.dims = (B, T, D, pd, npatch)
        ctx.pos_shape, ctx.cls_shape = pos.shape, cls_token.shape
        ctx.params = (weight, bias, cls_token, pos if pos.shape[-2:] == (T, D) and pos.is_leaf else None)
        chain_reset()
        return x

    @staticmethod
    @_scoped
    def backward(ctx, dx):
        (patches,) = ctx.saved_tensors
        B, T, D, pd, npatch = ctx.dims
        dx = _c(dx.float())
        weight, bias, cls_token, pos = ctx.params
        dpos, dcls, dy = ops.embed_bwd_gather(dx, B, T, D, patches.dtype, pos=pos, cls_token=cls_token)
        dw, db = ops.linear_dw(dy, patches, B * npatch, D, pd, weight=weight, bias=bias)
        return None, dw, db, dcls.view(ctx.cls_shape), dpos.view(ctx.pos_shape), None, None


def patch_embed(img, weight, bias, cls_token, pos, patch, prec):
    if img.requires_grad:
        raise RuntimeError("gradient w.r.t. the input image is not implemented (the reference never needs it)")
    return _PatchEmbed.apply(img, weight, bias, cls_token, pos, patch, prec)


_side = {}


def _publish_side(dx, dx16, colsum):
    _side.clear()
    _side[dx.data_ptr()] = (dx, dx16, colsum)


def _take_side(dout, rows, dim):
    ent = _side.pop(dout.data_ptr(), None)
    _side.clear()
    if ent is None or ent[0].shape != dout.shape or ent[1].shape[0] != rows or ent[1].shape[1] not in (dim, ops.current_segments() * dim):
        return None, None
    return ent[1], ent[2]


def _ln_bwd_with_side(dy, x, D, g, b, mean, rstd, dout, M, adt, up_bias=None):
    dx = torch.empty_like(x)
    if adt == torch.bfloat16:
        dx16 = torch.empty(M, D, dtype=torch.bfloat16, device=x.device)
        cs = ops.grad_out(up_bias, (D,), x.device)
        dg, db = ops.layernorm_bwd(dy, x, D, g, mean, rstd, dout, dx, D, M, D, dx16=dx16, dx_colsum=cs, beta=b)
        _publish_side(dx, dx16, cs)
    elif D <= 1024 and ops.x6_block_ok(M, D):
        dx6 = ops._split_buffer(M, D, x.device)
        cs = ops.grad_out(up_bias, (D,), x.device)
        dg, db = ops.layernorm_bwd(dy, x, D, g, mean, rstd, dout, dx, D, M, D, dx_split=dx6, dx_colsum=cs, beta=b)
        _publish_side(dx, dx6, cs)
    else:
        dg, db = ops.layernorm_bwd(dy, x, D, g, mean, rstd, dout, dx, D, M, D, beta=b)
    return dx, dg, db


_chain = [None]


def _chain_set(out, bias):
    _chain[0] = (weakref.ref(out), bias) if bias is not None else None


def _chain_take(x):
    c = _chain[0]
    return c[1] if c is not None and c[0]() is x else None


def chain_reset():
    _chain[0] = None



class _AttnBlock(Function):

    @staticmethod
    @_fwd
    def forward(ctx, x, g, b, wqkv, bqkv, wo, bo, heads, scale, prec):
        adt = ops.act_dtype(prec)
        B, T, D = x.shape
        M = B * T
        x = _c(x)
        ctx.up_bias = _chain_take(x)
        inner3 = wqkv.shape[0]
        inner = inner3 // 3
        ctx.x6 = adt == torch.float32 and ops.x6_block_ok(M, D, inner3, inner)
        if not (ctx.x6 and D <= 1024):
            y, mean, rstd = ops.layernorm_fwd(x, D, M, D, g, b, adt)
        if ctx.x6:
            dh = inner // heads
            y6, mean, rstd = ops.layernorm_fwd_split(x, D, M, D, g, b) if D <= 1024 else (ops.split_ex(y, M, D), mean, rstd)
            ctx.f16 = ops.attention_f16_supported(adt, T, dh)
            qkv = torch.empty(B, T, inner3, dtype=torch.float16 if ctx.f16 else adt, device=x.device)
            ops.nt_x6(y6, wqkv, "fwd", M, qkv.view(M, inner3), bias=bqkv)
            o = None
            if ctx.f16:
                o, probs = ops.attention_fwd_f16(qkv, B, T, heads, scale)
                ctx.fused32 = True
            elif ops.attention_f32_fused_supported(adt, T, dh):
                if any(ctx.needs_input_grad):
                    o, probs = ops.attention_fwd_f32_lse(qkv, B, T, heads, scale)
                else:
                    o, probs = ops.attention_fwd_f32(qkv, B, T, heads, scale), x.new_empty(0)
                ctx.fused32 = True
            else:
                probs = ops.attention_probs_fp32(qkv, B, T, heads, dh, scale)
                o = ops.attention_pv_fp32(probs, qkv, B, T, heads, dh)
                ctx.fused32 = False
            o6 = ops.split_ex(o.view(M, inner), M, inner)
            out = torch.empty_like(x)
            ops.nt_x6(o6, wo, "fwd", M, out.view(M, D), bias=bo, residual=x.view(M, D))
            ctx.save_for_backward(x, g, mean, rstd, y6, qkv, o6, probs, wqkv, wo, *((o,) if ctx.fused32 else ()))
            ctx.cfg = (heads, scale, False)
            ctx.small = (b, bqkv, bo)
            _chain_set(out, bo)
            return out
        qkv = torch.empty(B, T, inner3, dtype=adt, device=x.device)
        ops.linear_fwd(y, M, D, wqkv, bqkv, qkv, inner3)
        dh = inner // heads
        if ops.attention_fused_supported(adt, T, dh):
            o, lse = ops.attention_fwd(qkv, B, T, heads, scale)
            probs = None
        elif ops.attention_f32_fused_supported(adt, T, dh) and not any(ctx.needs_input_grad):
            o, lse, probs = ops.attention_fwd_f32(qkv, B, T, heads, scale), None, None
        elif ops.attention_f32_fused_supported(adt, T, dh):
            o, probs = ops.attention_fwd_f32_lse(qkv, B, T, heads, scale)
            lse, ctx.fused32 = None, True
        else:
            q32 = ops.cast(qkv, torch.float32)
            probs = ops.attention_probs_fp32(q32, B, T, heads, dh, scale)
            o = ops.cast(ops.attention_pv_fp32(probs, q32, B, T, heads, dh), adt)
            lse = None
        out = torch.empty_like(x)
        ops.linear_fwd(o.view(M, inner), M, inner, wo, bo, out, D, epi=EPI_RESIDUAL, aux=x, ld_aux=D)
        if lse is None and probs is None:
            probs = x.new_empty(0)
        ctx.save_for_backward(x, g, mean, rstd, y, qkv, o, lse if lse is not None else probs, wqkv, wo)
        ctx.cfg = (heads, scale, lse is not None)
        ctx.small = (b, bqkv, bo)
        _chain_set(out, bo)
        return out

    @staticmethod
    @_scoped
    def backward(ctx, dout):
        x, g, mean, rstd, y, qkv, o, lse_or_probs, wqkv, wo = ctx.saved_tensors[:10]
        heads, scale, fused = ctx.cfg
        B, T, D = x.shape
        M = B * T
        inner3 = wqkv.shape[0]
        inner = inner3 // 3
        if ctx.x6:
            y6, o6, probs = y, o, lse_or_probs
            dout = _c(dout)
            b, bqkv, bo = ctx.small
            d6, dbo = _take_side(dout, M, D)
            if d6 is None or d6.dtype != torch.bfloat16 or d6.shape[1] != ops.current_segments() * D:
                dbo = ops.grad_out(bo, (D,), x.device)
                d6 = ops.split_ex(dout.view(M, D), M, D, colsum_out=dbo)
            dwo = ops.tn_x6(d6, o6, M, wo)
            do = torch.empty(B, T, inner, dtype=torch.float32, device=x.device)
            ops.nt_x6(d6, wo, "dx", M, do.view(M, inner))
            dbqkv = ops.grad_out(bqkv, (inner3,), x.device)
            if ctx.f16:
                part = torch.empty(B, inner3, dtype=torch.float32, device=x.device)
                dq6 = ops.attention_bwd_f16(qkv, ctx.saved_tensors[10], do, probs, B, T, heads, scale, split=True, colsum=part)
                ops.colsum(part, B, inner3, inner3, dbqkv)
            else:
                if ctx.fused32:
                    dqkv = ops.attention_bwd_f32_fused(qkv, ctx.saved_tensors[10], do, probs, B, T, heads, scale)
                else:
                    dqkv = ops.attention_bwd_fp32(probs, qkv, do, B, T, heads, inner // heads, scale)
                dq6 = ops.split_ex(dqkv.view(M, inner3), M, inner3, colsum_out=dbqkv)
            dwqkv = ops.tn_x6(dq6, y6, M, wqkv)
            dy = torch.empty(M, D, dtype=torch.float32, device=x.device)
            ops.nt_x6(dq6, wqkv, "dx", M, dy)
            dx, dg, db = _ln_bwd_with_side(dy, x, D, g, b, mean, rstd, dout, M, torch.float32, ctx.up_bias)
            return dx, dg, db, dwqkv, dbqkv, dwo, dbo, None, None, None
        adt = y.dtype
        dout = _c(dout)
        d_act, dbo = _take_side(dout, M, D) if adt == torch.bfloat16 else (None, None)
        if d_act is None:
            d_act = ops.cast(dout, adt).view(M, D)
        b, bqkv, bo = ctx.small
        dwo, dbo2 = ops.linear_dw(d_act, o.view(M, inner), M, D, inner, want_bias=dbo is None, weight=wo, bias=bo)
        dbo = dbo if dbo is not None else dbo2
        do = torch.empty(B, T, inner, dtype=adt, device=x.device)
        ops.linear_dx(d_act, M, D, wo, do, inner)
        dbqkv = None
        if fused:
            part = torch.empty(B, inner3, dtype=torch.float32, device=x.device)
            dqkv = ops.attention_bwd(qkv, o, do, lse_or_probs, B, T, heads, scale, colsum=part)
            dbqkv = ops.colsum(part, B, inner3, inner3, ops.grad_out(bqkv, (inner3,), x.device))
        elif getattr(ctx, "fused32", False):
            dqkv = ops.attention_bwd_f32_fused(qkv, o, do, lse_or_probs, B, T, heads, scale)
        else:
            dqkv = ops.cast(ops.attention_bwd_fp32(lse_or_probs, ops.cast(qkv, torch.float32), ops.cast(do, torch.float32),
                                                   B, T, heads, inner // heads, scale), adt)
        dwqkv, dbq2 = ops.linear_dw(dqkv.view(M, inner3), y, M, inner3, D, want_bias=dbqkv is None, weight=wqkv, bias=bqkv)
        dbqkv = dbqkv if dbqkv is not None else dbq2
        dy = torch.empty(M, D, dtype=adt, device=x.device)
        ops.linear_dx(dqkv.view(M, inner3), M, inner3, wqkv, dy, D)
        dx, dg, db = _ln_bwd_with_side(dy, x, D, g, b, mean, rstd, dout, M, adt, ctx.up_bias)
        return dx, dg, db, dwqkv, dbqkv, dwo, dbo, None, None, None


def attn_block(x, g, b, wqkv, bqkv, wo, bo, heads, scale, prec):
    return _AttnBlock.apply(x, g, b, wqkv, bqkv, wo, bo, heads, scale, prec)


class _MlpBlock(Function):

    @staticmethod
    @_fwd
    def forward(ctx, x, g, b, w1, b1, w2, b2, prec):
        adt = ops.act_dtype(prec)
        B, T, D = x.shape
        M = B * T
        Hd = w1.shape[0]
        x = _c(x)
        ctx.up_bias = _chain_take(x)
        ctx.x6 = adt == torch.float32 and ops.x6_block_ok(M, D, Hd)
        if not (ctx.x6 and D <= 1024):
            y, mean, rstd = ops.layernorm_fwd(x, D, M, D, g, b, adt)
        if ctx.x6:
            y6, mean, rstd = ops.layernorm_fwd_split(x, D, M, D, g, b) if D <= 1024 else (ops.split_ex(y, M, D), mean, rstd)
            h = torch.empty(M, Hd, dtype=adt, device=x.device)
            if ops.nt_split_ok(M, Hd, D):
                a6 = ops.nt_x6_gelu_split(y6, w1, M, h, bias=b1)
            else:
                ops.nt_x6(y6, w1, "fwd", M, h, bias=b1)
                a6 = ops.split_ex(h, M, Hd, op=1)
            out = torch.empty_like(x)
            ops.nt_x6(a6, w2, "fwd", M, out.view(M, D), bias=b2, residual=x.view(M, D))
            ctx.save_for_backward(x, g, mean, rstd, y6, h, a6, w1, w2)
            ctx.small = (b, b1, b2)
            _chain_set(out, b2)
            return out
        g8 = adt == torch.bfloat16 and GELU_GRAD_BITS == 8 and Hd % 8 == 0
        h = torch.empty(M, Hd, dtype=torch.uint8 if g8 else adt, device=x.device)
        a = torch.empty(M, Hd, dtype=adt, device=x.device)
        ops.linear_fwd(y, M, D, w1, b1, a, Hd, epi=(EPI_GELU_GRAD8 if g8 else EPI_GELU_GRAD) if adt == torch.bfloat16 else EPI_GELU,
                       out2=h, ld_out2=Hd)
        out = torch.empty_like(x)
        ops.linear_fwd(a, M, Hd, w2, b2, out, D, epi=EPI_RESIDUAL, aux=x, ld_aux=D)
        ctx.save_for_backward(x, g, mean, rstd, y, h, a, w1, w2)
        ctx.small = (b, b1, b2)
        _chain_set(out, b2)
        return out

    @staticmethod
    @_scoped
    def backward(ctx, dout):
        x, g, mean, rstd, y, h, a, w1, w2 = ctx.saved_tensors
        B, T, D = x.shape
        M = B * T
        Hd = w1.shape[0]
        if ctx.x6:
            y6, a6 = y, a
            dout = _c(dout)
            b, b1, b2 = ctx.small
            d6, db2 = _take_side(dout, M, D)
            if d6 is None or d6.dtype != torch.bfloat16 or d6.shape[1] != ops.current_segments() * D:
                db2 = ops.grad_out(b2, (D,), x.device)
                d6 = ops.split_ex(dout.view(M, D), M, D, colsum_out=db2)
            dw2 = ops.tn_x6(d6, a6, M, w2)
            db1 = ops.grad_out(b1, (Hd,), x.device)
            if ops.nt_split_ok(M, Hd, D):
                dh6 = ops.nt_x6_dgelu_split(d6, w2, M, h, db1)
            else:
                dh = torch.empty(M, Hd, dtype=torch.float32, device=x.device)
                ops.nt_x6(d6, w2, "dx", M, dh)
                dh6 = ops.split_ex(dh, M, Hd, op=2, h=h, colsum_out=db1)
            dw1 = ops.tn_x6(dh6, y6, M, w1)
            dy = torch.empty(M, D, dtype=torch.float32, device=x.device)
            ops.nt_x6(dh6, w1, "dx", M, dy)
            dx, dg, db = _ln_bwd_with_side(dy, x, D, g, b, mean, rstd, dout, M, torch.float32, ctx.up_bias)
            return dx, dg, db, dw1, db1, dw2, db2, None
        adt = y.dtype
        dout = _c(dout)
        d_act, db2 = _take_side(dout, M, D) if adt == torch.bfloat16 else (None, None)
        if d_act is None:
            d_act = ops.cast(dout, adt).view(M, D)
        b, b1, b2 = ctx.small
        dw2, db2b = ops.linear_dw(d_act, a, M, D, Hd, want_bias=db2 is None, weight=w2, bias=b2)
        db2 = db2 if db2 is not None else db2b
        dh = torch.empty(M, Hd, dtype=adt, device=x.device)
        if adt == torch.bfloat16:
            part = torch.empty((M + 63) // 64, Hd, dtype=torch.float32, device=x.device)
            ops.linear_dx(d_act, M, D, w2, dh, Hd, epi=EPI_MUL8 if h.dtype == torch.uint8 else EPI_MUL, aux=h, ld_aux=Hd,
                          colsum_partial=part)
            db1 = ops.colsum(part, part.shape[0], Hd, Hd, ops.grad_out(b1, (Hd,), x.device))
            dw1, _ = ops.linear_dw(dh, y, M, Hd, D, want_bias=False, weight=w1)
        else:
            ops.linear_dx(d_act, M, D, w2, dh, Hd, epi=EPI_DGELU, aux=h, ld_aux=Hd)
            dw1, db1 = ops.linear_dw(dh, y, M, Hd, D, weight=w1, bias=b1)
        dy = torch.empty(M, D, dtype=adt, device=x.device)
        ops.linear_dx(dh, M, Hd, w1, dy, D)
        dx, dg, db = _ln_bwd_with_side(dy, x, D, g, b, mean, rstd, dout, M, adt, ctx.up_bias)
        return dx, dg, db, dw1, db1, dw2, db2, None


def mlp_block(x, g, b, w1, b1, w2, b2, prec):
    return _MlpBlock.apply(x, g, b, w1, b1, w2, b2, prec)


class _ClsHead(Function):

    @staticmethod
    @_fwd
    def forward(ctx, x, g, b, w, bias, prec):
        adt = ops.act_dtype(prec)
        B, T, D = x.shape
        C = w.shape[0]
        x = _c(x)
        y, mean, rstd = ops.layernorm_fwd(x, T * D, B, D, g, b, adt)
        logits = torch.empty(B, C, dtype=torch.float32, device=x.device)
        ops.linear_fwd(y, B, D, w, bias, logits, C)
        ctx.save_for_backward(x, g, mean, rstd, y, w)
        ctx.small = (b, bias)
        return logits

    @staticmethod
    @_scoped
    def backward(ctx, dlogits):
        x, g, mean, rstd, y, w = ctx.saved_tensors
        B, T, D = x.shape
        C = w.shape[0]
        adt = y.dtype
        ld = ops.pad8(C) if adt == torch.bfloat16 else C
        dl = torch.zeros(B, ld, dtype=adt, device=x.device)
        dl[:, :C] = dlogits
        b, bias = ctx.small
        dw, dbias = ops.linear_dw(dl, y, B, C, D, ld_dy=ld, weight=w, bias=bias)
        dy = torch.empty(B, D, dtype=adt, device=x.device)
        ops.linear_dx(dl, B, C, w, dy, D, ld_dy=ld)
        dx = torch.zeros_like(x)
        dg, db = ops.layernorm_bwd(dy, x, T * D, g, mean, rstd, None, dx, T * D, B, D, beta=b)
        return dx, dg, db, dw, dbias, None


def cls_head(x, g, b, w, bias, prec):
    return _ClsHead.apply(x, g, b, w, bias, prec)


def _seg_small_fwd(x, g, b, w, bias, prec):
    adt = ops.act_dtype(prec)
    B, T, D = x.shape
    C = w.shape[0]
    npatch = T - 1
    x = _c(x)
    xp = ops.gather_patch_rows(x, B, T, D, torch.float32)
    M = B * npatch
    y, mean, rstd = ops.layernorm_fwd(xp, D, M, D, g, b, adt)
    small = torch.empty(M, C, dtype=torch.float32, device=x.device)
    ops.linear_fwd(y, M, D, w, bias, small, C)
    return small, (xp, g, mean, rstd, y, w), (b, bias)


def _seg_small_bwd(saved, small_params, dims, dl, ld):
    xp, g, mean, rstd, y, w = saved
    b, bias = small_params
    B, T, D, C = dims
    npatch = T - 1
    M = B * npatch
    adt = y.dtype
    dw, dbias = ops.linear_dw(dl, y, M, C, D, ld_dy=ld, weight=w, bias=bias)
    dy = torch.empty(M, D, dtype=adt, device=dl.device)
    ops.linear_dx(dl, M, C, w, dy, D, ld_dy=ld)
    dx = torch.zeros(B, T, D, dtype=torch.float32, device=dl.device)
    dxp = torch.empty(M, D, dtype=torch.float32, device=dl.device)
    dg, db = ops.layernorm_bwd(dy, xp, D, g, mean, rstd, None, dxp, D, M, D, beta=b)
    dx[:, 1:, :] = dxp.view(B, npatch, D)
    return dx, dg, db, dw, dbias


class _UpsampleBilinear(Function):

    @staticmethod
    @_fwd
    def forward(ctx, small, grid, size):
        ops.require_cuda(small)
        B, hw, C = small.shape
        small = _c(small.float())
        ctx.dims = (B, C, grid, size)
        return ops.upsample_bilinear_fwd(small, hw * C, 1, C, B, C, grid, grid, size, size)

# ... 137 lines not shown
```

### myrtle-vision_amd/myrtle_vision/hip/lib.py

```python
import ctypes
import os
import threading

import torch

from .build import LIB_PATH

MV_F32, MV_BF16, MV_I8, MV_F16 = 0, 1, 2, 3
EPI_NONE, EPI_GELU, EPI_RESIDUAL, EPI_DGELU, EPI_EMBED, EPI_GELU_GRAD, EPI_MUL, EPI_GELU_Q8 = 0, 1, 2, 3, 4, 5, 6, 7
EPI_GELU_GRAD8, EPI_MUL8, EPI_SPLIT_DGELU, EPI_SPLIT_GELU = 8, 9, 10, 11

_P, _I, _L, _F, _Z = ctypes.c_void_p, ctypes.c_int, ctypes.c_long, ctypes.c_float, ctypes.c_size_t
_KIND = {"p": _P, "i": _I, "l": _L, "f": _F, "z": _Z, "Q": ctypes.c_uint64}

SIGNATURES = {
    "mv_version": ("", _I),
    "mv_error_string": ("i", ctypes.c_char_p),
    "mv_gemm_tn_workspace_bytes": ("iii", _Z),
    "mv_layernorm_bwd_workspace_bytes": ("ii", _Z),
    "mv_layernorm_fwd": ("plpppipp" "iifp", _I),
    "mv_layernorm_fwd_split": ("plpppipp" "iifp", _I),
    "mv_layernorm_bwd": ("pi" "plp" "pp" "ppl" "ppi" "pz" "ii" "pp" "p", _I),
    "mv_layernorm_bwd_split": ("pi" "plp" "pp" "ppl" "ppi" "pz" "ii" "pip" "p", _I),
    "mv_gemm_nt_bf16": ("pipipii" "iii" "pi" "pii" "pi" "p", _I),
    "mv_gemm_nt_bf16_scaled": ("pipipii" "iii" "f" "pi" "pii" "pi" "p", _I),
    "mv_quant_affine_codes": ("pip" "lii" "f" "iiii" "p", _I),
    "mv_quant_float_f16": ("pp" "l" "p", _I),
    "mv_gemm_nt_f16": ("pipipi" "iii" "p" "i" "pi" "pi" "p", _I),
    "mv_quant_affine_i8": ("pip" "lii" "f" "ii" "p", _I),
    "mv_gemm_nt_i8": ("pipipii" "iii" "f" "pp" "i" "pi" "fi" "p", _I),
    "mv_layernorm_fwd_q8": ("plppp" "ii" "ff" "i" "p", _I),
    "mv_attention_fwd_f32_q8": ("pp" "iii" "f" "f" "i" "p", _I),
    "mv_gemm_tn_bf16": ("pipipi" "iii" "i" "p" "pz" "p", _I),
    "mv_gemm_f32": ("pllll" "pllll" "pllll" "iii" "ii" "fi" "pi" "pli" "pl" "p", _I),
    "mv_attention_bwd_force": ("i", _I),
    "mv_attention_fwd_force": ("i", _I),
    "mv_attention_fwd_f32_lse": ("ppp" "iii" "f" "p", _I),
    "mv_attention_bwd_f32": ("ppppp" "iii" "f" "p", _I),
    "mv_gemm_f32_force_fma": ("i", _I),
    "mv_sum_slabs": ("pli" "pli" "p", _I),
    "mv_sum_slabs_add": ("pli" "ppl" "p", _I),
    "mv_gemm_nt_bf16_ksplit": ("pipip" "iiii" "p" "p", _I),
    "mv_attention_fwd": ("ppp" "iii" "f" "p", _I),
    "mv_attention_bwd": ("pppppp" "iii" "f" "p", _I),
    "mv_attention_fwd_f32": ("pp" "iii" "f" "p", _I),
    "mv_attention_fwd_f16": ("ppp" "iii" "f" "p", _I),
    "mv_attention_bwd_prep_f16": ("ppppp" "iii" "p", _I),
    "mv_attention_bwd_f16": ("pppppp" "ip" "iii" "f" "p", _I),
    "mv_softmax_fwd": ("pp" "li" "f" "p", _I),
    "mv_softmax_bwd": ("ppp" "li" "f" "p", _I),
    "mv_patchify": ("ppi" "iiiii" "p", _I),
    "mv_embed_cls": ("ppp" "iii" "p", _I),
    "mv_embed_bwd": ("ppp" "i" "iii" "p", _I),
    "mv_gather_patch_rows": ("ppi" "iii" "p", _I),
    "mv_embed_bwd_gather": ("ppi" "pp" "iii" "p", _I),
    "mv_cast": ("pipi" "l" "p", _I),
    "mv_split3_bf16": ("plpll" "lii" "p", _I),
    "mv_split3_ex_workspace_bytes": ("li", _Z),
    "mv_split3_bf16_ex": ("plpl" "ip" "li" "ppz" "p", _I),
    "mv_gemm_tn_bf16_x6": ("ppp" "iiii" "pz" "p", _I),
    "mv_split2_bf16": ("plpll" "lii" "p", _I),
    "mv_weight_split": ("ppp" "iii" "p", _I),
    "mv_split_f8c": ("plpl" "liii" "p", _I),
    "mv_gemm_nt_f8c": ("plplpi" "iiiii" "pipi" "p", _I),
    "mv_split2_bf16_ex": ("plpl" "ip" "li" "ppz" "p", _I),
    "mv_gemm_tn_bf16_x3": ("ppp" "iiii" "pz" "p", _I),
    "mv_weight_prep": ("ppipi" "ii" "p", _I),
    "mv_weight_prep_batch": ("pii" "p", _I),
    "mv_colsum": ("pil" "pi" "li" "pz" "p", _I),
    "mv_gelu_fwd": ("ppi" "l" "p", _I),
    "mv_gelu_bwd": ("pppi" "l" "p", _I),
    "mv_add_f32": ("ppp" "l" "p", _I),
    "mv_quant_float": ("pp" "l" "ii" "p", _I),
    "mv_quant_fixed": ("pp" "l" "iiii" "p", _I),
    "mv_quant_affine": ("pp" "l" "f" "iii" "p", _I),
    "mv_minmax": ("pl" "p" "p", _I),
    "mv_cross_entropy": ("ppp" "pii" "p" "lil" "f" "p", _I),
    "mv_upsample_bilinear_fwd": ("plll" "p" "iiiiii" "p", _I),
    "mv_upsample_bilinear_bwd": ("pplll" "iiiiii" "p", _I),
    "mv_gemm_force_variant": ("ii", _I),
    "mv_seg_ce_partials": ("iii", _L),
    "mv_seg_ce_fwd": ("pppppp" "iiiiii" "p", _I),
    "mv_seg_ce_bwd": ("ppppp" "ii" "f" "iiiiii" "p", _I),
    "mv_image_prepare": ("plii" "pppp" "i" "p" "ffffff" "p" "iii" "p", _I),
    "mv_mask_prepare": ("plii" "pp" "p" "i" "p" "iii" "p", _I),
    "mv_image_resize_u8": ("plii" "pppp" "i" "p" "iii" "p", _I),
    "mv_mask_resize_u8": ("plii" "pp" "p" "iii" "p", _I),
    "mv_adamw": ("pppp" "l" "ffffffff" "p" "p", _I),
    "mv_adamw_dev": ("pppp" "l" "p" "fffff" "p" "p", _I),
    "mv_grad_norm_workspace_bytes": ("", _Z),
    "mv_grad_norm_clip": ("pl" "ff" "p" "pz" "p", _I),
    "mv_dropout": ("ppi" "l" "f" "QQ" "p", _I),
}

_lock = threading.Lock()
_lib = None


class HipLibraryMissing(RuntimeError):
    pass


def lib():
    global _lib
    if _lib is None:
        with _lock:
            if _lib is None:
                if not os.path.exists(LIB_PATH):
# ... 18 lines not shown
```

### myrtle-vision_amd/myrtle_vision/hip/ops.py

```python
import ctypes
import os
import threading
import weakref

import torch

from . import lib as _l
from .lib import (EPI_DGELU, EPI_EMBED, EPI_GELU, EPI_GELU_GRAD, EPI_GELU_GRAD8, EPI_MUL, EPI_MUL8, EPI_NONE, EPI_RESIDUAL,
                  EPI_SPLIT_DGELU, EPI_SPLIT_GELU, MV_BF16, MV_F32, check,
                  lib)

__all__ = ["EPI_NONE", "EPI_GELU", "EPI_RESIDUAL", "EPI_DGELU", "EPI_EMBED", "EPI_GELU_GRAD", "EPI_MUL", "EPI_GELU_GRAD8", "EPI_MUL8",
           "EPI_SPLIT_DGELU", "EPI_SPLIT_GELU"]

_DT = {torch.float32: MV_F32, torch.bfloat16: MV_BF16}


def act_dtype(prec: str):
    if prec == "bf16":
        return torch.bfloat16
    if prec in ("fp32", "bf16x3", "bf16x3h"):
        return torch.float32
    raise ValueError(f"unknown precision {prec!r} (expected 'bf16', 'bf16x3', 'bf16x3h' or 'fp32')")


def require_cuda(*tensors):
    for t in tensors:
        if t is not None and not t.is_cuda:
            raise RuntimeError(
                "myrtle_vision computes only through its HIP kernels on an MI355X: got a CPU tensor "
                "(there is no CPU fallback; move the model and inputs to 'cuda')")


def _s():
    return torch.cuda.current_stream().cuda_stream


def _p(t):
    return None if t is None else t.data_ptr()


def pad8(n: int) -> int:
    return (n + 7) & ~7


class KernelTimer:

    def __init__(self, sample_every: int = 1, sample_steps=None):
        self.records = {}
        self.by_shape = {}
        self.sample_every = max(int(sample_every), 1)
        self.sample_steps = None if sample_steps is None else set(int(s) for s in sample_steps)
        self.step = -1
        self.active = True

    def next_step(self):
        self.step += 1
        self.active = (self.step in self.sample_steps) if self.sample_steps is not None else self.step % self.sample_every == 0

    def begin(self):
        if not self.active:
            return None
        e = torch.cuda.Event(enable_timing=True)
        e.record()
        return e

    def end(self, name, start, flops, shape=None):
        if start is None:
            return
        e = torch.cuda.Event(enable_timing=True)
        e.record()
        self.records.setdefault(name, []).append((start, e, flops))
        if shape is not None:
            self.by_shape.setdefault(shape, []).append((start, e, flops))

    def shape_summary(self):
        torch.cuda.synchronize()
        out = {}
        for shape, recs in self.by_shape.items():
            ms = sum(s.elapsed_time(e) for s, e, _ in recs)
            out[shape] = dict(launches=len(recs), avg_us=1e3 * ms / len(recs),
                              tflops=sum(f for _, _, f in recs) / (ms * 1e-3) / 1e12 if ms > 0 else 0.0)
        return out

    def summary(self):
        torch.cuda.synchronize()
        out = {}
        for name, recs in self.records.items():
            ms = sum(s.elapsed_time(e) for s, e, _ in recs)
            fl = sum(f for _, _, f in recs)
            out[name] = dict(launches=len(recs), total_ms=ms, avg_us=1e3 * ms / len(recs), flops_per_launch=fl / len(recs),
                             tflops=fl / (ms * 1e-3) / 1e12 if ms > 0 else 0.0)
# ... 439 lines not shown
    if t0 is not None:
        _timer.end(f"gemm_nt_bf16x{nseg}", t0, 2.0 * M * N * K, shape=f"dx N{K} K{N} split-dgelu")
    colsum(part, part.shape[0], K, K, colsum_out)
    return dh6


def tn_x6(dy6, x6, M, weight):
    N, K = weight.shape
    dw = grad_out(weight, (N, K), dy6.device)
    _tn_segments(dy6, x6, dw, M, N, K)
    return dw


def _tn_segments(dy6, x6, dw, M, N, K):
    nseg = current_segments()
    Mp = pad32(M)
    ws = workspace(lib().mv_gemm_tn_workspace_bytes(N, K, nseg * Mp), dy6.device)
    t0 = _timer.begin() if _timer is not None else None
    fn = lib().mv_gemm_tn_bf16_x6 if nseg == 6 else lib().mv_gemm_tn_bf16_x3
    check(fn(_p(dy6), _p(x6), _p(dw), K, N, K, Mp, _p(ws), ws.numel(), _s()), f"gemm_tn_bf16_x{nseg}", M=N, N=K, rows=Mp)
    if t0 is not None:
        _timer.end(f"gemm_tn_bf16x{nseg}", t0, 2.0 * M * N * K, shape=f"dw N{N} K{K}")


def _x6_ksplits(M, N):
    tiles = ((M + 255) // 256) * ((N + 255) // 256)
    r1, r3 = -(-tiles // 256), -(-(3 * tiles) // 256) / 3.0
    return 3 if r3 <= 0.75 * r1 else 1


def _nt_x6(a6, b6, out, ldc, M, N, Kc, bias, epi, aux=None, ld_aux=0, aux_i=0, tag="fwd"):
    nseg = current_segments()
    Kx = nseg * Kc
    t0 = _timer.begin() if _timer is not None else None
    S = _x6_ksplits(M, N) if epi in (EPI_NONE, EPI_RESIDUAL) and ldc == N and (aux is None or ld_aux == N) else 1
    if S > 1 and (Kx % (128 * S) != 0 or out.dtype != torch.float32):
        S = 1
    c_dt = MV_F32 if out.dtype == torch.float32 else _l.MV_F16
    if S > 1:
        slabs = workspace(S * M * N * 4, out.device)
        check(lib().mv_gemm_nt_bf16_ksplit(_p(a6), Kx, _p(b6), Kx, _p(slabs), M, N, Kx, S, _p(bias), _s()),
              f"gemm_nt_bf16_ksplit(x{nseg})", M=M, N=N, K=Kx, S=S)
        check(lib().mv_sum_slabs_add(_p(slabs), M * N, S, _p(aux) if epi == EPI_RESIDUAL else None, _p(out), M * N, _s()),
              "sum_slabs_add", n=M * N)
        if t0 is not None:
            _timer.end(f"gemm_nt_bf16x{nseg}", t0, 2.0 * M * N * Kc, shape=f"{tag} N{N} K{Kc} epi{epi} S{S}")
        return
    check(lib().mv_gemm_nt_bf16(_p(a6), Kx, _p(b6), Kx, _p(out), ldc, c_dt, M, N, Kx, _p(bias), epi, _p(aux),
                                ld_aux, aux_i, None, 0, _s()), f"gemm_nt_bf16(x{nseg})", M=M, N=N, K=Kx, epi=epi)
    if t0 is not None:
        _timer.end(f"gemm_nt_bf16x{nseg}", t0, 2.0 * M * N * Kc, shape=f"{tag} N{N} K{Kc} epi{epi}")


def linear_fwd(x, M, K, weight, bias, out, ldc, *, lda=None, epi=EPI_NONE, aux=None, ld_aux=0, aux_i=0, out2=None,
               ld_out2=0):
    N = weight.shape[0]
    lda = K if lda is None else lda
    if x.dtype == torch.bfloat16:
        pw = prepared_weight(weight)
        t0 = _timer.begin() if _timer is not None else None
        check(lib().mv_gemm_nt_bf16(_p(x), lda, _p(pw.w), pw.ldw, _p(out), ldc, _DT[out.dtype], M, N, K, _p(bias), epi,
                                    _p(aux), ld_aux, aux_i, _p(out2), ld_out2, _s()),
              "gemm_nt_bf16", M=M, N=N, K=K, epi=epi)
        if t0 is not None:
            _timer.end("gemm_nt_bf16", t0, 2.0 * M * N * K, shape=f"fwd N{N} K{K} epi{epi}")
    elif (_x6_nt_ok(M, N, K) and out.dtype == torch.float32 and weight.dtype == torch.float32
          and (epi in (EPI_NONE, EPI_RESIDUAL, EPI_EMBED) and out2 is None
               or epi == EPI_GELU and ldc == N and (out2 is None or ld_out2 == N))):
        a6, b6 = split_act(x, M, K, lda), split_weight(weight, "fwd")
        if epi == EPI_GELU:
            pre = out if out2 is None else out2
            _nt_x6(a6, b6, pre, N, M, N, K, bias, EPI_NONE)
            check(lib().mv_gelu_fwd(_p(pre), _p(out), MV_F32, M * N, _s()), "gelu_fwd", n=M * N)
        else:
            _nt_x6(a6, b6, out, ldc, M, N, K, bias, epi, aux, ld_aux, aux_i)
    else:
        w = weight.detach()
        check(lib().mv_gemm_f32(_p(x), lda, 1, 0, 0, _p(w), 1, w.stride(0), 0, 0, _p(out), ldc, 1, 0, 0, M, N, K, 1, 1,
                                1.0, 0, _p(bias), epi, _p(aux), ld_aux, aux_i, _p(out2), ld_out2, _s()),
              "gemm_f32", M=M, N=N, K=K, epi=epi)
    return out


def linear_dx(dy, M, N, weight, out, ldc, *, ld_dy=None, epi=EPI_NONE, aux=None, ld_aux=0, colsum_partial=None):
    K = weight.shape[1]
    ld_dy = N if ld_dy is None else ld_dy
    if dy.dtype == torch.bfloat16:
        pw = prepared_weight(weight)
        t0 = _timer.begin() if _timer is not None else None
        check(lib().mv_gemm_nt_bf16(_p(dy), ld_dy, _p(pw.wt), pw.ldt, _p(out), ldc, _DT[out.dtype], M, K, N, None, epi,
                                    _p(aux), ld_aux, 0, _p(colsum_partial), K if colsum_partial is not None else 0, _s()),
              "gemm_nt_bf16(dx)", M=M, N=K, K=N, epi=epi)
        if t0 is not None:
            _timer.end("gemm_nt_bf16", t0, 2.0 * M * N * K, shape=f"dx N{K} K{N} epi{epi}")
    elif (_x6_nt_ok(M, K, N) and out.dtype == torch.float32 and weight.dtype == torch.float32
          and (epi == EPI_NONE or epi == EPI_DGELU and ldc == K and ld_aux == K)):
        _nt_x6(split_act(dy, M, N, ld_dy), split_weight(weight, "dx"), out, ldc, M, K, N, None, EPI_NONE, tag="dx")
        if epi == EPI_DGELU:
            check(lib().mv_gelu_bwd(_p(aux), _p(out), _p(out), MV_F32, M * K, _s()), "gelu_bwd", n=M * K)
    else:
        w = weight.detach()
        check(lib().mv_gemm_f32(_p(dy), ld_dy, 1, 0, 0, _p(w), w.stride(0), 1, 0, 0, _p(out), ldc, 1, 0, 0, M, K, N, 1,
                                1, 1.0, 0, None, epi, _p(aux), ld_aux, 0, None, 0, _s()),
              "gemm_f32(dx)", M=M, N=K, K=N, epi=epi)
    return out


def linear_dw(dy, x, M, N, K, *, ld_dy=None, ldx=None, want_bias=True, weight=None, bias=None):
    ld_dy = N if ld_dy is None else ld_dy
    ldx = K if ldx is None else ldx
    dw = grad_out(weight, (N, K), x.device)
    db = grad_out(bias, (N,), x.device) if want_bias else None
    if dy.dtype == torch.bfloat16:
        nbytes = lib().mv_gemm_tn_workspace_bytes(N, K, M)
        ws = workspace(nbytes, x.device)
        t0 = _timer.begin() if _timer is not None else None
        check(lib().mv_gemm_tn_bf16(_p(dy), ld_dy, _p(x), ldx, _p(dw), K, N, K, M, 0, _p(db), _p(ws), ws.numel(), _s()),
              "gemm_tn_bf16", M=N, N=K, Kc=M)
        if t0 is not None:
            _timer.end("gemm_tn_bf16(+reduce+colsum)", t0, 2.0 * M * N * K, shape=f"dw N{N} K{K} bias{int(want_bias)}")
    elif _x6_tn_ok(M, N, K) and dy.dtype == torch.float32 and x.dtype == torch.float32:
        a6, b6 = split_act(dy, M, N, ld_dy, colsum_out=db if want_bias else None), split_act(x, M, K, ldx)
        _tn_segments(a6, b6, dw, M, N, K)
    else:
        S = f32_dw_splits(M, N, K)
        if S == 1:
            check(lib().mv_gemm_f32(_p(dy), 1, ld_dy, 0, 0, _p(x), ldx, 1, 0, 0, _p(dw), K, 1, 0, 0, N, K, M, 1, 1, 1.0, 0,
                                    None, EPI_NONE, None, 0, 0, None, 0, _s()), "gemm_f32(dw)", M=N, N=K, K=M)
        else:
            Mc = M // S
            slabs = workspace(S * N * K * 4, x.device).view(torch.float32)[:S * N * K]
            check(lib().mv_gemm_f32(_p(dy), 1, ld_dy, Mc * ld_dy, 0, _p(x), ldx, 1, Mc * ldx, 0, _p(slabs), K, 1, N * K, 0,
                                    N, K, Mc, S, 1, 1.0, 0, None, EPI_NONE, None, 0, 0, None, 0, _s()),
                  "gemm_f32(dw, split)", M=N, N=K, K=Mc, S=S)
            check(lib().mv_sum_slabs(_p(slabs), N * K, S, _p(dw), N * K, 0, _s()), "sum_slabs", S=S, n=N * K)
        if want_bias:
            colsum(dy, M, N, ld_dy, db)
    return dw, db


def f32_dw_splits(M, N, K):
    tiles = ((N + 127) // 128) * ((K + 127) // 128)
    best = 1
    for s in (2, 4, 8, 16, 32):
        if M % (16 * s) == 0 and M // s >= 512 and tiles * best < 512 and (N * K) % 4 == 0:
            best = s
    return best


def colsum(x, rows, cols, ld, out):
    ws = workspace(256 * cols * 4 + 1024, x.device)
    check(lib().mv_colsum(_p(x), _DT[x.dtype], ld, _p(out), 0, rows, cols, _p(ws), ws.numel(), _s()), "colsum",
          rows=rows, cols=cols)
    return out


def attention_fused_supported(qkv_dtype, N, dim_head):
    return qkv_dtype == torch.bfloat16 and dim_head == 64 and N <= 320


def attention_fwd(qkv, B, N, H, scale):
    require_cuda(qkv)
    out = torch.empty(B, N, H * 64, dtype=torch.bfloat16, device=qkv.device)
    lse = torch.empty(B, H, N, dtype=torch.float32, device=qkv.device)
    check(lib().mv_attention_fwd(_p(qkv), _p(out), _p(lse), B, N, H, scale, _s()), "attention_fwd", B=B, N=N, H=H)
    return out, lse
# ... 461 lines not shown
```

### myrtle-vision_amd/myrtle_vision/models/vit.py

```python
import os
from contextlib import nullcontext
from typing import Optional, Union

import torch
import torch.autograd.profiler as profiler
import torch.nn.functional as TF
from torch import nn

from myrtle_vision.hip import functional as F
from myrtle_vision.hip import ops
from myrtle_vision.utils.quantize import DeQuantStub, FloatFunctional, ModelQuantizer, QFormat, QuantStub

MIN_NUM_PATCHES = 16


def _default_precision() -> str:
    return os.environ.get("MYRTLE_VISION_PRECISION", "bf16")


class _HipModule:

    precision = "bf16"

    @property
    def act_dtype(self):
        return ops.act_dtype(self.precision)


class Linear(nn.Linear, _HipModule):

    def forward(self, x):
        ops.require_cuda(x, self.weight)
        if x.dtype != self.act_dtype:
            x = F.cast(x, self.act_dtype)
        with ops.segments(ops.prec_segments(self.precision)):
            return F.linear(x, self.weight, self.bias)


class LayerNorm(nn.LayerNorm, _HipModule):
    def forward(self, x):
        ops.require_cuda(x, self.weight)
        return F.layer_norm(x, self.weight, self.bias, self.act_dtype, self.eps)


class GELU(nn.GELU, _HipModule):
    def forward(self, x):
        ops.require_cuda(x)
        return F.gelu(x)


class Dropout(nn.Dropout):

    def forward(self, x):
        return F.dropout(x, self.p, self.training)


def _plain(module, cls):
    return type(module) is cls and not module._forward_hooks and not module._forward_pre_hooks


def _int8_linear(m):
    if isinstance(m, nn.Sequential) and len(m) == 2 and getattr(m[0], "passthrough", False):
        if m._forward_hooks or m._forward_pre_hooks or m[0]._forward_hooks or m[0]._forward_pre_hooks:
            return None
        m = m[1]
    if type(m).__name__ != "Int8Linear" or m._forward_hooks or m._forward_pre_hooks:
        return None
    return m


def _int8_fusable(x, norm, first, second, M):
    return (type(first).fuse_quant and not (torch.is_grad_enabled() and x.requires_grad) and x.is_cuda
            and x.dtype == torch.float32 and _plain(norm, LayerNorm) and norm.weight.shape[0] % 16 == 0
            and norm.weight.shape[0] <= 1024 and first.takes_codes(M) and second.takes_codes(M))


class Residual(nn.Module):
    def __init__(self, fn: nn.Module):
        super().__init__()
        self.fn = fn
        self.res_add = FloatFunctional()

    def forward(self, x: torch.Tensor):
        fused = self._fused(x)
        if fused is not None:
            return fused
        return self.res_add.add(self.fn(x), x)

    def _fusable_plain(self):
        pn = self.fn
        return (type(pn) is PreNorm and _plain(pn.norm, LayerNorm) and self.res_add.plain() and not self._forward_hooks
                and not self._forward_pre_hooks and not pn._forward_hooks and not pn._forward_pre_hooks
                and type(pn.fn) is FeedForward and pn.fn.fusable() and not pn.fn._forward_hooks and not pn.fn._forward_pre_hooks)

    def _fused(self, x):
        pn = self.fn
        if not (type(pn) is PreNorm and _plain(pn.norm, LayerNorm) and self.res_add.plain()):
            return None
        if pn._forward_hooks or pn._forward_pre_hooks or x.dim() != 3:
            return None
        ops.require_cuda(x)
        inner = pn.fn
        prec = pn.norm.precision
        x = x.float()
        if type(inner) is Attention and inner.fusable():
            lin_o = inner.to_out[0]
            return F.attn_block(x, pn.norm.weight, pn.norm.bias, inner.to_qkv.weight, inner.to_qkv.bias, lin_o.weight,
                                lin_o.bias, inner.heads, inner.scale, prec)
        if type(inner) is FeedForward and inner.fusable():
            fc1, fc2 = inner.net[0], inner.net[3]
            return F.mlp_block(x, pn.norm.weight, pn.norm.bias, fc1.weight, fc1.bias, fc2.weight, fc2.bias, prec)
        if type(inner) is Attention and inner.int8_pair() is not None:
            fused = inner.int8_fused_forward(x, pn.norm)
            return fused if fused is not None else inner.int8_forward(pn.norm(x), residual=x)
        if type(inner) is FeedForward and inner.int8_pair() is not None:
            fused = inner.int8_fused_forward(x, pn.norm)
            if fused is not None:
                return fused
            fc1, fc2 = inner.int8_pair()
            return fc2(fc1(pn.norm(x)), pre_gelu=True, residual=x)
        return None


class PreNorm(nn.Module):
    def __init__(self, dim: int, fn: nn.Module):
        super().__init__()
        self.norm = LayerNorm(dim)
        self.fn = fn

    def forward(self, x: torch.Tensor):
        return self.fn(self.norm(x))


class FeedForward(nn.Module):
    def __init__(self, dim: int, hidden_dim: int, dropout: float = 0.0):
        super().__init__()
        self.net = nn.Sequential(
            Linear(dim, hidden_dim),
            GELU(),
            Dropout(dropout),
            Linear(hidden_dim, dim),
            Dropout(dropout),
        )

    def fusable(self):
        n = self.net
        return (not self._forward_hooks and not n._forward_hooks and _plain(n[0], Linear) and _plain(n[1], GELU)
                and _plain(n[3], Linear) and all(type(n[i]) is Dropout and (n[i].p == 0.0 or not n[i].training)
                                                 and not n[i]._forward_hooks for i in (2, 4)))

    def int8_pair(self):
        n = self.net
        fc1, fc2 = _int8_linear(n[0]), _int8_linear(n[3])
        if (fc1 is not None and fc2 is not None and _plain(n[1], GELU) and not self._forward_hooks
                and not n._forward_hooks and not n._forward_pre_hooks
                and all(type(n[i]) is Dropout and (n[i].p == 0.0 or not n[i].training) and not n[i]._forward_hooks
                        for i in (2, 4))):
            return fc1, fc2
        return None

    def int8_fused_forward(self, x, norm):
        fc1, fc2 = self.int8_pair()
        B, T, D = x.shape
        M = B * T
        if (not _int8_fusable(x, norm, fc1, fc2, M)) or M % 256 != 0 or fc1.weight.shape[0] % 256 != 0:
            return None
        x = x.contiguous()
        x8 = ops.layernorm_q8(x, D, M, D, norm.weight, norm.bias, norm.eps, *fc1.qparams)
        h8 = fc1.forward_codes(x8, M, gelu_q8=fc2.qparams)
        return fc2.forward_codes(h8, M, residual=x).view(B, T, D)

    def forward(self, x: torch.Tensor):
        pair = self.int8_pair()
        if pair is not None:
            return pair[1](pair[0](x), pre_gelu=True)
        return self.net(x)


class Attention(nn.Module):
    def __init__(self, dim: int, heads: int = 8, dim_head: int = 64, dropout: float = 0.0):
        super().__init__()
        inner_dim = dim_head * heads
        self.heads = heads
        self.scale = dim_head ** -0.5

        self.to_qkv = Linear(dim, inner_dim * 3, bias=True)
        self.to_out = nn.Sequential(
            Linear(inner_dim, dim),
            Dropout(dropout),
        )

        self.dequant_qkv = DeQuantStub()
        self.quant_out = QuantStub()
        self.bf16_core = False
        self.attn_output = nn.Identity()

    def fusable(self):
        d = self.to_out[1]
        return (not self._forward_hooks and _plain(self.to_qkv, Linear) and _plain(self.to_out[0], Linear)
                and not self.to_out._forward_hooks and type(d) is Dropout and (d.p == 0.0 or not d.training)
                and not self.attn_output._forward_hooks and self.dequant_qkv.plain() and self.quant_out.plain())

    def int8_pair(self):
        lq, lo = _int8_linear(self.to_qkv), _int8_linear(self.to_out[0])
        d = self.to_out[1]
        if (lq is not None and lo is not None and not self._forward_hooks and not self.to_out._forward_hooks
                and type(d) is Dropout and (d.p == 0.0 or not d.training) and not d._forward_hooks
                and not self.attn_output._forward_hooks and self.dequant_qkv.plain() and self.quant_out.plain()):
            return lq, lo
        return None

    def int8_fused_forward(self, x, norm):
        lq, lo = self.int8_pair()
        B, T, D = x.shape
        M = B * T
        dh = lq.weight.shape[0] // (3 * self.heads)
        if (not _int8_fusable(x, norm, lq, lo, M)) or self.bf16_core or not ops.attention_f32_fused_supported(torch.float32, T, dh):
            return None
        x = x.contiguous()
        x8 = ops.layernorm_q8(x, D, M, D, norm.weight, norm.bias, norm.eps, *lq.qparams)
        qkv = lq.forward_codes(x8, M)
        o8 = ops.attention_fwd_f32_q8(qkv, B, T, self.heads, self.scale, *lo.qparams)
        return lo.forward_codes(o8.view(M, -1), M, residual=x).view(B, T, D)

    def int8_forward(self, x, residual=None):
        lq, lo = self.int8_pair()
        qkv = lq(x, out_dtype=torch.bfloat16 if self.bf16_core else torch.float32)
        return lo(F.attention_core(qkv, self.heads, self.scale, None), residual=residual)

    def forward(self, x: torch.Tensor):
        if self.int8_pair() is not None:
            return self.int8_forward(x)
        qkv = self.dequant_qkv(self.to_qkv(x))
        hook = self.attn_output if self.attn_output._forward_hooks else None
        if self.bf16_core and hook is None and qkv.dtype == torch.float32:
            out = F.cast(F.attention_core(F.cast(qkv, torch.bfloat16), self.heads, self.scale, None), torch.float32)
        else:
            out = F.attention_core(qkv, self.heads, self.scale, hook)
        out = self.quant_out(out)
        out = self.to_out(out)
        return out


class Transformer(nn.Module):
    def __init__(self, dim: int, depth: int, heads: int, dim_head: int, mlp_dim: int, dropout: float, profile: bool):
        super().__init__()
        if profile:
            self.cm_attention = profiler.record_function("transformer:attention")
            self.cm_feedforward = profiler.record_function("transformer:feedforward")
        else:
            self.cm_attention = nullcontext()
            self.cm_feedforward = nullcontext()

        self.layers = nn.ModuleList([])
        for _ in range(depth):
            self.layers.append(
                nn.Sequential(
                    Residual(PreNorm(dim, Attention(dim, heads=heads, dim_head=dim_head, dropout=dropout))),
                    Residual(PreNorm(dim, FeedForward(dim, mlp_dim, dropout=dropout))),
                )
            )

    cls_only_tail = False

    def _tail_prunable(self, blk):
        ff = blk[1]
        return (self.cls_only_tail and ff._fusable_plain() and not blk._forward_hooks and not blk._forward_pre_hooks)

    def forward(self, x: torch.Tensor):
        last = len(self.layers) - 1
        for i, transformer_block in enumerate(self.layers):
            with self.cm_attention:
                x = transformer_block[0](x)
            with self.cm_feedforward:
                if i == last and x.dim() == 3 and self._tail_prunable(transformer_block):
                    x = x[:, :1]
                x = transformer_block[1](x)
        return x


class ViT(nn.Module):
    def __init__(
        self,
        *,
        decoder: str,
        image_size: int,
        patch_size: int,
        num_classes: int,
        dim: int,
        depth: int,
        heads: int,
        mlp_dim: int,
        pool: str = "cls",
        channels: int = 3,
        dim_head: int = 64,
        dropout: float = 0.0,
        emb_dropout: float = 0.0,
        num_det_tokens: int = 100,
        profile: bool = False,
        q_format: Optional[Union[str, QFormat]] = None,
        precision: Optional[str] = None,
        prune_dead_tokens: Optional[bool] = None,
    ):
        super().__init__()
        assert image_size % patch_size == 0, "Image dimensions must be divisible by the patch size."
        num_patches = (image_size // patch_size) ** 2
        patch_dim = channels * patch_size ** 2
        assert num_patches > MIN_NUM_PATCHES, (
            f"your number of patches ({num_patches}) is way too small for "
            f"attention to be effective (at least 16). Try decreasing your "
            f"patch size"
        )
        assert decoder in {
            "classification",
            "segmentation",
            "detection",
        }, "decoder must be either classification, segmentation, or detection"
        if heads * dim_head != dim:
            raise ValueError(f"heads * dim_head must equal dim (got {heads} * {dim_head} != {dim})")
        self.patch_size = patch_size

        if profile:
            self.cm_patch_to_embedding = profiler.record_function("patch_to_embedding")
            self.cm_transformer = profiler.record_function("transformer")
            self.cm_mlp_head = profiler.record_function("mlp_head")
        else:
            self.cm_patch_to_embedding = nullcontext()
            self.cm_transformer = nullcontext()
            self.cm_mlp_head = nullcontext()

        self.pos_embedding = nn.Parameter(torch.randn(1, 14 * 14 + 1, dim))
        self.pos_embedding_det = nn.Parameter(torch.randn(1, num_det_tokens, dim))
        self.patch_to_embedding = Linear(patch_dim, dim)
        self.cls_token = nn.Parameter(torch.randn(1, 1, dim))
        self.det_tokens = nn.Parameter(torch.randn(1, num_det_tokens, dim))
        self.dropout = Dropout(emb_dropout)

        self.transformer = Transformer(dim, depth, heads, dim_head, mlp_dim, dropout, profile)
        if prune_dead_tokens is None:
            prune_dead_tokens = os.environ.get("MYRTLE_VISION_PRUNE_DEAD_TOKENS", "0") == "1"
        self.transformer.cls_only_tail = bool(prune_dead_tokens) and decoder == "classification"

        if decoder == "classification":
            self.decoder = ClassificationDecoder(dim, num_classes)
        elif decoder == "segmentation":
            self.decoder = SegmentationDecoder(dim, num_classes, image_size, patch_size)
        elif decoder == "detection":
            self.decoder = DetectionDecoder(dim, num_classes, num_det_tokens)

        self.quant_img = QuantStub()
        self.quant_pos_embedding = QuantStub()
        self.quant_cls_token = QuantStub()
        self.quant_det_tokens = QuantStub()
        self.dequant_output = DeQuantStub()
        self.cls_token_cat = FloatFunctional()
        self.pos_embedding_add = FloatFunctional()
        self.pos_embedding_cat = FloatFunctional()
        self.set_precision(precision if precision is not None else _default_precision())
        self.quantizer = ModelQuantizer(self)
        self.quantizer.prepare_qat(q_format if q_format is not None else QFormat.FP32)
# ... 165 lines not shown
```

Before: 7271.

## Fuse next block's LayerNorm into residual GEMM epilogue via row-completion counters

Adds an MV_EPI_RESIDUAL_LN epilogue to the 8-phase NT GEMM. Each tile writes its residual output, then atomically bumps a per-128-row counter, and the last tile to finish a row band computes LayerNorm over the full 768-wide rows, emitting bf16 y, mean and rstd. The goal is to remove the separate LayerNorm launch and its re-read of the residual stream before the next attention or MLP block, with the model forward threading the next block's gamma and beta through. In exchange, the last CTA per band does serialized tail work, it relies on atomics and fences for cross-tile visibility, and outputs are stored with a cache-bypass store; only N=768 and M%128==0 are supported, otherwise it falls back.

```diff
diff --git a/include/myrtle_vision_hip.h b/include/myrtle_vision_hip.h
--- a/include/myrtle_vision_hip.h
+++ b/include/myrtle_vision_hip.h
@@ -33,6 +33,7 @@
   MV_EPI_MUL8 = 9,
   MV_EPI_SPLIT_DGELU = 10,
   MV_EPI_SPLIT_GELU = 11,
+  MV_EPI_RESIDUAL_LN = 12,
   MV_EPI_EMBED = 4
 };
 
@@ -61,6 +62,11 @@
 int mv_gemm_nt_bf16_scaled(const void* A, int lda, const void* B, int ldb, void* C, int ldc, int c_dtype, int M, int N,
                            int K, float alpha, const float* bias, int epilogue, const void* aux, int ld_aux, int aux_i,
                            void* out2, int ld_out2, mv_stream_t stream);
+int mv_gemm_nt_ln_counters(int M);
+int mv_gemm_nt_ln_init(int* counters, int n, mv_stream_t stream);
+int mv_gemm_nt_bf16_ln(const void* A, int lda, const void* B, int ldb, float* C, int ldc, int M, int N, int K, const float* bias,
+                       const float* aux, int ld_aux, const float* gamma, const float* beta, float eps, void* y, float* mean,
+                       float* rstd, int* counters, mv_stream_t stream);
 int mv_gemm_tn_bf16(const void* A, int lda, const void* B, int ldb, float* C, int ldc, int M, int N, int Kc,
                     int accumulate, float* colsum, float* workspace, size_t workspace_bytes, mv_stream_t stream);
 
diff --git a/myrtle-vision_amd/csrc/gemm_bf16.hip b/myrtle-vision_amd/csrc/gemm_bf16.hip
--- a/myrtle-vision_amd/csrc/gemm_bf16.hip
+++ b/myrtle-vision_amd/csrc/gemm_bf16.hip
@@ -1,4 +1,5 @@
 #include "mv_common.h"
+#include "layernorm_row.h"
 
 #include <atomic>
 #include <type_traits>
@@ -33,6 +34,13 @@
   long ks_slab;
   int band;
   int f8_tiles16, f8_scale;
+  const float* ln_gamma;
+  const float* ln_beta;
+  float ln_eps;
+  bf16_t* ln_y;
+  float* ln_mean;
+  float* ln_rstd;
+  int* ln_count;
 };
 
 __device__ __forceinline__ void st16(void* p, u32x4 v) { *reinterpret_cast<u32x4*>(p) = v; }
@@ -170,7 +178,7 @@
   return interior && EPI == MV_EPI_RESIDUAL;
 }
 
-template <int EPI, typename CT, bool PRE = false>
+template <int EPI, typename CT, bool PRE = false, bool SC1 = false>
 __device__ __forceinline__ void nt_epilogue(f32x4 (&acc)[4][4], CT* __restrict__ C, int ldc, int M, int N, int m0, int n0,
                                             int wm, int wn, int lane, const EpiArgs& ep, const float* bias_lds = nullptr,
                                             const EpiPre<EPI>& pre = EpiPre<EPI>{}) {
@@ -379,6 +387,10 @@
         }
         if constexpr (epi_is_split(EPI))
           store_pieces4(reinterpret_cast<bf16_t*>(C) + crow[i] * ldc + n, v, ep.aux_i, N);
+        else if constexpr (SC1)
+          __builtin_amdgcn_raw_buffer_store_b128(__builtin_bit_cast(u32x4, (f32x4){v[0], v[1], v[2], v[3]}),
+                                                 __builtin_amdgcn_make_buffer_rsrc(C, (short)0, 0x7FFFFFFF, 0x00020000),
+                                                 (int)((crow[i] * ldc + n) * (long)sizeof(CT)), 0, 16);
         else if constexpr (sizeof(CT) == 4)
           st16(C + crow[i] * ldc + n, __builtin_bit_cast(u32x4, (f32x4){v[0], v[1], v[2], v[3]}));
         else
@@ -777,6 +789,50 @@
 typedef __attribute__((ext_vector_type(8))) int i32x8;
 typedef __attribute__((ext_vector_type(8))) _Float16 f16x8;
 
+typedef __attribute__((address_space(1))) int g_int;
+constexpr int LN_EPI_N = 768, LN_EPI_VPL = LN_EPI_N / 256;
+__device__ __forceinline__ void nt_ln_rows(const float* C, int ldc, int r0, int wave, int lane, const EpiArgs& ep) {
+#pragma unroll 1
+  for (int b = 0; b < 2; ++b) {
+    const long rb = r0 + wave * 16 + b * 8;
+    float4 v[8][LN_EPI_VPL];
+#pragma unroll
+    for (int r = 0; r < 8; ++r) ln_row_load<LN_EPI_VPL>(C + (rb + r) * ldc, lane, LN_EPI_N / 4, v[r]);
+#pragma unroll
+    for (int r = 0; r < 8; ++r)
+      ln_row_fwd<LN_EPI_VPL, bf16_t>(v[r], lane, LN_EPI_N, ep.ln_eps, ep.ln_gamma, ep.ln_beta, ep.ln_y + (rb + r) * LN_EPI_N,
+                                     ep.ln_mean, ep.ln_rstd, rb + r);
+  }
+}
+__device__ __forceinline__ void nt_ln_tail(const float* C, int ldc, int M, int tiles_n, int t, int half, int tid, int lane, int wave,
+                                           char* smem, const EpiArgs& ep) {
+  const int hp = (t / tiles_n) * 2 + (half >= 0 ? half : 0);
+  const int nh = half >= 0 ? 1 : 2;
+  asm volatile("s_waitcnt vmcnt(0)" ::: "memory");
+  __syncthreads();
+  int* const flag = reinterpret_cast<int*>(smem);
+  if (tid == 0) {
+    int last = 0;
+    for (int k = 0; k < nh; ++k) {
+      if ((hp + k) * 128 >= M) break;
+      g_int* const cnt = (g_int*)(ep.ln_count + hp + k);
+      if (__hip_atomic_fetch_add(cnt, 1, __ATOMIC_RELAXED, __HIP_MEMORY_SCOPE_AGENT) == tiles_n - 1) {
+        __hip_atomic_store(cnt, 0, __ATOMIC_RELAXED, __HIP_MEMORY_SCOPE_AGENT);
+        last |= 1 << k;
+      }
+    }
+    if (last) {
+      __builtin_amdgcn_fence(__ATOMIC_ACQUIRE, "agent");
+      asm volatile("s_waitcnt vmcnt(0)" ::: "memory");
+    }
+    flag[0] = last;
+  }
+  __syncthreads();
+  const int last = flag[0];
+  for (int k = 0; k < nh; ++k)
+    if (last & (1 << k)) nt_ln_rows(C, ldc, (hp + k) * 128, wave, lane, ep);
+}
+
 template <int EPI, typename CT, int OPK = NT_BF16, bool KSPLIT = false>
 __global__ __launch_bounds__(512, 2) void gemm_nt_8phase_kernel(const bf16_t* __restrict__ A, int lda,
                                                                 const bf16_t* __restrict__ B, int ldb, CT* __restrict__ C,
@@ -804,6 +860,8 @@
     half = idx & 1;
   }
   const bool is_half_rt = half >= 0;
+  constexpr bool LNT = EPI == MV_EPI_RESIDUAL_LN;
+  constexpr int EPIX = LNT ? MV_EPI_RESIDUAL : EPI;
   if constexpr (KSPLIT) {
     const int ks = t / ep.ks_tiles;
     t -= ks * ep.ks_tiles;
@@ -1025,7 +1083,7 @@
       }
     }
   }
-  constexpr bool park = epi_is_dgelu(EPI) || EPI == MV_EPI_RESIDUAL || EPI == MV_EPI_SPLIT_DGELU;
+  constexpr bool park = epi_is_dgelu(EPIX) || EPIX == MV_EPI_RESIDUAL || EPIX == MV_EPI_SPLIT_DGELU;
   f32x4* const parked = reinterpret_cast<f32x4*>(smem) + wave * 16 * 64 + lane;
   if (park && !is_half) {
 #pragma unroll
@@ -1033,24 +1091,24 @@
 #pragma unroll
       for (int j = 0; j < 4; ++j) parked[(i * 4 + j) * 64] = acc[4 + i][j];
   }
-  constexpr bool can_pre = (EPI == MV_EPI_RESIDUAL || EPI == MV_EPI_MUL8) && !KSPLIT;
+  constexpr bool can_pre = (EPIX == MV_EPI_RESIDUAL || EPIX == MV_EPI_MUL8) && !KSPLIT;
   if constexpr (can_pre) {
-    if (!is_half && nt_epi_prefetch_ok<EPI>(M, N, m0 + 128 * wm, n0 + 128 * (wn >> 1), ldc, ep)) {
-      EpiPre<EPI> pre0, pre1;
-      nt_epi_prefetch<EPI>(pre0, m0 + 128 * wm, n0 + 128 * (wn >> 1), 0, wn & 1, lane, ep);
-      nt_epi_prefetch<EPI>(pre1, m0 + 128 * wm, n0 + 128 * (wn >> 1), 1, wn & 1, lane, ep);
-      nt_epilogue<EPI, CT, true>(*reinterpret_cast<f32x4(*)[4][4]>(&acc[0]), C, ldc, M, N, m0 + 128 * wm, n0 + 128 * (wn >> 1), 0,
+    if (!is_half && nt_epi_prefetch_ok<EPIX>(M, N, m0 + 128 * wm, n0 + 128 * (wn >> 1), ldc, ep)) {
+      EpiPre<EPIX> pre0, pre1;
+      nt_epi_prefetch<EPIX>(pre0, m0 + 128 * wm, n0 + 128 * (wn >> 1), 0, wn & 1, lane, ep);
+      nt_epi_prefetch<EPIX>(pre1, m0 + 128 * wm, n0 + 128 * (wn >> 1), 1, wn & 1, lane, ep);
+      nt_epilogue<EPIX, CT, true, LNT>(*reinterpret_cast<f32x4(*)[4][4]>(&acc[0]), C, ldc, M, N, m0 + 128 * wm, n0 + 128 * (wn >> 1), 0,
                                  wn & 1, lane, ep, nullptr, pre0);
       f32x4 accb[4][4];
 #pragma unroll
       for (int i = 0; i < 4; ++i)
 #pragma unroll
         for (int j = 0; j < 4; ++j) accb[i][j] = parked[(i * 4 + j) * 64];
-      nt_epilogue<EPI, CT, true>(accb, C, ldc, M, N, m0 + 128 * wm, n0 + 128 * (wn >> 1), 1, wn & 1, lane, ep, nullptr, pre1);
+      nt_epilogue<EPIX, CT, true, LNT>(accb, C, ldc, M, N, m0 + 128 * wm, n0 + 128 * (wn >> 1), 1, wn & 1, lane, ep, nullptr, pre1);
       return;
     }
   }
-  nt_epilogue<EPI, CT>(*reinterpret_cast<f32x4(*)[4][4]>(&acc[0]), C, ldc, M, N, is_half ? m0 : m0 + 128 * wm,
+  nt_epilogue<EPIX, CT, false, LNT>(*reinterpret_cast<f32x4(*)[4][4]>(&acc[0]), C, ldc, M, N, is_half ? m0 : m0 + 128 * wm,
                        n0 + 128 * (wn >> 1), is_half ? wm : 0, wn & 1, lane, ep);
   if (is_half) return;
   f32x4 acc2[4][4];
@@ -1065,10 +1123,11 @@
 #pragma unroll
       for (int j = 0; j < 4; ++j) acc2[i][j] = acc[4 + i][j];
   }
-  nt_epilogue<EPI, CT>(acc2, C, ldc, M, N, m0 + 128 * wm, n0 + 128 * (wn >> 1), 1, wn & 1, lane, ep);
+  nt_epilogue<EPIX, CT, false, LNT>(acc2, C, ldc, M, N, m0 + 128 * wm, n0 + 128 * (wn >> 1), 1, wn & 1, lane, ep);
   };
   if (is_half_rt) body(std::true_type{});
   else body(std::false_type{});
+  if constexpr (LNT) nt_ln_tail(reinterpret_cast<const float*>(C), ldc, M, tiles_n, t, half, tid, lane, wave, smem, ep);
 }
 
 __device__ __forceinline__ void tn_store(f32x4 (&acc)[4][4], float* __restrict__ Cs, long ldc, int M, int N, int m0, int n0,
@@ -1567,9 +1626,12 @@
 template <int EPI, typename CT>
 int launch_nt(const void* A, int lda, const void* B, int ldb, void* C, int ldc, int M, int N, int K, EpiArgs ep,
               hipStream_t s) {
-  const int attr = MV_ONCE_PER_DEVICE(set_smem(gemm_nt_kernel<EPI, CT>) | set_smem(gemm_nt_glds_kernel<EPI, CT>) |
-                          set_smem(gemm_nt_glds_kernel<EPI, CT, false>));
-  if (attr != 0) return MV_ERR_LAUNCH;
+  constexpr bool p8_only = EPI == MV_EPI_RESIDUAL_LN;
+  if constexpr (!p8_only) {
+    const int attr = MV_ONCE_PER_DEVICE(set_smem(gemm_nt_kernel<EPI, CT>) | set_smem(gemm_nt_glds_kernel<EPI, CT>) |
+                            set_smem(gemm_nt_glds_kernel<EPI, CT, false>));
+    if (attr != 0) return MV_ERR_LAUNCH;
+  }
   const int tiles_m = mv_cdiv(M, BM), tiles_n = mv_cdiv(N, BN);
   const int t2m = mv_cdiv(M, BM2), t2n = mv_cdiv(N, BN2);
   int force = g_force_nt.load(std::memory_order_relaxed);
@@ -1599,6 +1661,9 @@
     MV_CHECK_LAUNCH();
     return MV_OK;
   }
+  if constexpr (p8_only) {
+    return MV_ERR_UNSUPPORTED;
+  } else {
   if ((force == 2564 && ring_ok) || (force == 0 && ring_pick)) {
     const int a4 = MV_ONCE_PER_DEVICE(hipFuncSetAttribute(reinterpret_cast<const void*>(gemm_nt_ring_kernel<EPI, CT, 4>),
                                               hipFuncAttributeMaxDynamicSharedMemorySize, 4 * RSTAGE_BYTES) == hipSuccess ? 0 : -1);
@@ -1618,6 +1683,12 @@
                                                                         (CT*)C, ldc, M, N, K, tiles_n, ep);
   MV_CHECK_LAUNCH();
   return MV_OK;
+  }
+}
+
+__global__ void ln_epi_zero_kernel(int* __restrict__ c, int n) {
+  const int i = blockIdx.x * blockDim.x + threadIdx.x;
+  if (i < n) c[i] = 0;
 }
 
 }
@@ -1689,6 +1760,39 @@
   }
 }
 
+extern "C" int mv_gemm_nt_ln_counters(int M) { return M > 0 ? mv_cdiv(M, 128) : 0; }
+
+extern "C" int mv_gemm_nt_ln_init(int* counters, int n, mv_stream_t stream) {
+  MV_REQUIRE(n >= 0, MV_ERR_SHAPE);
+  if (n == 0) return MV_OK;
+  ln_epi_zero_kernel<<<mv_cdiv(n, 256), 256, 0, (hipStream_t)stream>>>(counters, n);
+  MV_CHECK_LAUNCH();
+  return MV_OK;
+}
+
+extern "C" int mv_gemm_nt_bf16_ln(const void* A, int lda, const void* B, int ldb, float* C, int ldc, int M, int N, int K,
+                                  const float* bias, const float* aux, int ld_aux, const float* gamma, const float* beta, float eps,
+                                  void* y, float* mean, float* rstd, int* counters, mv_stream_t stream) {
+  MV_REQUIRE(M >= 0 && K >= 0, MV_ERR_SHAPE);
+  if (M == 0) return MV_OK;
+  if (N != LN_EPI_N || M % 128 != 0 || ldc % 4 != 0 || ld_aux % 4 != 0 || ldc < N || (long)M * ldc * 4 >= (1L << 31) ||
+      (bias && !mv_aligned16(bias)))
+    return MV_ERR_UNSUPPORTED;
+  MV_REQUIRE(lda % 8 == 0 && ldb % 8 == 0 && lda >= ((K + 7) & ~7) && ldb >= ((K + 7) & ~7), MV_ERR_ALIGN);
+  MV_REQUIRE(mv_aligned16(A) && mv_aligned16(B) && mv_aligned16(C) && aux && mv_aligned16(aux), MV_ERR_ALIGN);
+  MV_REQUIRE(gamma && beta && y && mean && rstd && counters && mv_aligned16(gamma) && mv_aligned16(beta) && mv_aligned16(y),
+             MV_ERR_ALIGN);
+  EpiArgs ep{1.0f, bias, aux, ld_aux, 0, nullptr, 0, nullptr, 0.f, 0.f};
+  ep.ln_gamma = gamma;
+  ep.ln_beta = beta;
+  ep.ln_eps = eps;
+  ep.ln_y = (bf16_t*)y;
+  ep.ln_mean = mean;
+  ep.ln_rstd = rstd;
+  ep.ln_count = counters;
+  return launch_nt<MV_EPI_RESIDUAL_LN, float>(A, lda, B, ldb, C, ldc, M, N, K, ep, (hipStream_t)stream);
+}
+
 extern "C" int mv_gemm_nt_bf16_ksplit(const void* A, int lda, const void* B, int ldb, float* slabs, int M, int N, int K,
                                       int splits, const float* bias, mv_stream_t stream) {
   MV_REQUIRE(M > 0 && N > 0 && K > 0 && splits >= 1, MV_ERR_SHAPE);
diff --git a/myrtle-vision_amd/csrc/layernorm.hip b/myrtle-vision_amd/csrc/layernorm.hip
--- a/myrtle-vision_amd/csrc/layernorm.hip
+++ b/myrtle-vision_amd/csrc/layernorm.hip
@@ -1,4 +1,5 @@
 #include "mv_common.h"
+#include "layernorm_row.h"
 
 namespace {
 
@@ -10,67 +11,10 @@
                                                      int dim, float eps, float q_inv = 0.f, float q_zp = 0.f) {
   const int lane = threadIdx.x & 63;
   const int wave = threadIdx.x >> 6;
-  const int nvec = dim >> 2;
-  const float inv_dim = 1.0f / (float)dim;
   for (long row = (long)blockIdx.x * 4 + wave; row < rows; row += (long)gridDim.x * 4) {
-    const float4* xr = reinterpret_cast<const float4*>(x + row * ldx);
     float4 v[VPL];
-    float s = 0.f;
-#pragma unroll
-    for (int i = 0; i < VPL; ++i) {
-      const int c = lane + 64 * i;
-      v[i] = (c < nvec) ? xr[c] : make_float4(0.f, 0.f, 0.f, 0.f);
-      s += (v[i].x + v[i].y) + (v[i].z + v[i].w);
-    }
-    const float mu = wave_sum(s) * inv_dim;
-    float q = 0.f;
-#pragma unroll
-    for (int i = 0; i < VPL; ++i) {
-      const int c = lane + 64 * i;
-      if (c < nvec) {
-        const float a = v[i].x - mu, b = v[i].y - mu, cc = v[i].z - mu, d = v[i].w - mu;
-        q += (a * a + b * b) + (cc * cc + d * d);
-      }
-    }
-    const float rs = rsqrtf(wave_sum(q) * inv_dim + eps);
-    if (lane == 0 && mean) {
-      mean[row] = mu;
-      rstd[row] = rs;
-    }
-    YT* yr = y + row * (long)dim * (NSEG ? NSEG : 1);
-#pragma unroll
-    for (int i = 0; i < VPL; ++i) {
-      const int c = lane + 64 * i;
-      if (c < nvec) {
-        const float4 g = reinterpret_cast<const float4*>(gamma)[c];
-        const float4 b = reinterpret_cast<const float4*>(beta)[c];
-        const float o0 = (v[i].x - mu) * rs * g.x + b.x, o1 = (v[i].y - mu) * rs * g.y + b.y;
-        const float o2 = (v[i].z - mu) * rs * g.z + b.z, o3 = (v[i].w - mu) * rs * g.w + b.w;
-        if constexpr (NSEG != 0) {
-          const float o[4] = {o0, o1, o2, o3};
-          bf16x4 p[3];
-#pragma unroll
-          for (int e = 0; e < 4; ++e) {
-            const bf16_t p0 = (bf16_t)o[e];
-            const float r1 = o[e] - (float)p0;
-            const bf16_t p1 = (bf16_t)r1;
-            p[0][e] = p0;
-            p[1][e] = p1;
-            p[2][e] = (bf16_t)(r1 - (float)p1);
-          }
-          constexpr int order[6] = {0, 0, 1, 0, 1, 2};
-#pragma unroll
-          for (int sgm = 0; sgm < NSEG; ++sgm) reinterpret_cast<bf16x4*>(yr + (long)sgm * dim)[c] = p[order[sgm]];
-        } else if constexpr (sizeof(YT) == 1) {
-          reinterpret_cast<unsigned*>(yr)[c] = affine_i8_pack4<0>(o0, o1, o2, o3, q_inv, q_zp);
-        } else if constexpr (sizeof(YT) == 4) {
-          reinterpret_cast<float4*>(yr)[c] = make_float4(o0, o1, o2, o3);
-        } else {
-          bf16x4 o = {(bf16_t)o0, (bf16_t)o1, (bf16_t)o2, (bf16_t)o3};
-          reinterpret_cast<bf16x4*>(yr)[c] = o;
-        }
-      }
-    }
+    ln_row_load<VPL>(x + row * ldx, lane, dim >> 2, v);
+    ln_row_fwd<VPL, YT, NSEG>(v, lane, dim, eps, gamma, beta, y + row * (long)dim * (NSEG ? NSEG : 1), mean, rstd, row, q_inv, q_zp);
   }
 }
 
diff --git a/myrtle-vision_amd/csrc/layernorm_row.h b/myrtle-vision_amd/csrc/layernorm_row.h
--- /dev/null
+++ b/myrtle-vision_amd/csrc/layernorm_row.h
@@ -0,0 +1,72 @@
+#pragma once
+#include "mv_common.h"
+
+template <int VPL>
+__device__ __forceinline__ void ln_row_load(const float* xr, int lane, int nvec, float4 (&v)[VPL]) {
+  const float4* x4 = reinterpret_cast<const float4*>(xr);
+#pragma unroll
+  for (int i = 0; i < VPL; ++i) {
+    const int c = lane + 64 * i;
+    v[i] = (c < nvec) ? x4[c] : make_float4(0.f, 0.f, 0.f, 0.f);
+  }
+}
+
+template <int VPL, typename YT, int NSEG = 0>
+__device__ __forceinline__ void ln_row_fwd(const float4 (&v)[VPL], int lane, int dim, float eps, const float* __restrict__ gamma,
+                                           const float* __restrict__ beta, YT* __restrict__ yr, float* __restrict__ mean,
+                                           float* __restrict__ rstd, long row, float q_inv = 0.f, float q_zp = 0.f) {
+#pragma clang fp contract(off)
+  const int nvec = dim >> 2;
+  const float inv_dim = 1.0f / (float)dim;
+  float s = 0.f;
+#pragma unroll
+  for (int i = 0; i < VPL; ++i) s += (v[i].x + v[i].y) + (v[i].z + v[i].w);
+  const float mu = wave_sum(s) * inv_dim;
+  float q = 0.f;
+#pragma unroll
+  for (int i = 0; i < VPL; ++i) {
+    const int c = lane + 64 * i;
+    if (c < nvec) {
+      const float a = v[i].x - mu, b = v[i].y - mu, cc = v[i].z - mu, d = v[i].w - mu;
+      q += __builtin_fmaf(a, a, b * b) + __builtin_fmaf(cc, cc, d * d);
+    }
+  }
+  const float rs = rsqrtf(__builtin_fmaf(wave_sum(q), inv_dim, eps));
+  if (lane == 0 && mean) {
+    mean[row] = mu;
+    rstd[row] = rs;
+  }
+#pragma unroll
+  for (int i = 0; i < VPL; ++i) {
+    const int c = lane + 64 * i;
+    if (c < nvec) {
+      const float4 g = reinterpret_cast<const float4*>(gamma)[c];
+      const float4 b = reinterpret_cast<const float4*>(beta)[c];
+      const float o0 = __builtin_fmaf((v[i].x - mu) * rs, g.x, b.x), o1 = __builtin_fmaf((v[i].y - mu) * rs, g.y, b.y);
+      const float o2 = __builtin_fmaf((v[i].z - mu) * rs, g.z, b.z), o3 = __builtin_fmaf((v[i].w - mu) * rs, g.w, b.w);
+      if constexpr (NSEG != 0) {
+        const float o[4] = {o0, o1, o2, o3};
+        bf16x4 p[3];
+#pragma unroll
+        for (int e = 0; e < 4; ++e) {
+          const bf16_t p0 = (bf16_t)o[e];
+          const float r1 = o[e] - (float)p0;
+          const bf16_t p1 = (bf16_t)r1;
+          p[0][e] = p0;
+          p[1][e] = p1;
+          p[2][e] = (bf16_t)(r1 - (float)p1);
+        }
+        constexpr int order[6] = {0, 0, 1, 0, 1, 2};
+#pragma unroll
+        for (int sgm = 0; sgm < NSEG; ++sgm) reinterpret_cast<bf16x4*>(yr + (long)sgm * dim)[c] = p[order[sgm]];
+      } else if constexpr (sizeof(YT) == 1) {
+        reinterpret_cast<unsigned*>(yr)[c] = affine_i8_pack4<0>(o0, o1, o2, o3, q_inv, q_zp);
+      } else if constexpr (sizeof(YT) == 4) {
+        reinterpret_cast<float4*>(yr)[c] = make_float4(o0, o1, o2, o3);
+      } else {
+        bf16x4 o = {(bf16_t)o0, (bf16_t)o1, (bf16_t)o2, (bf16_t)o3};
+        reinterpret_cast<bf16x4*>(yr)[c] = o;
+      }
+    }
+  }
+}
diff --git a/myrtle-vision_amd/myrtle_vision/hip/functional.py b/myrtle-vision_amd/myrtle_vision/hip/functional.py
--- a/myrtle-vision_amd/myrtle_vision/hip/functional.py
+++ b/myrtle-vision_amd/myrtle_vision/hip/functional.py
@@ -1,4 +1,5 @@
 import functools
+import os
 import weakref
 
 import torch
@@ -10,6 +11,7 @@
 
 
 GELU_GRAD_BITS = 8
+LN_EPILOGUE = os.environ.get("MV_LN_EPILOGUE", "0") == "1"
 
 
 def _c(t):
@@ -452,6 +454,28 @@
 
 def chain_reset():
     _chain[0] = None
+    _ln_next[0] = None
+
+
+_ln_next = [None]
+
+
+def _residual_out(a, M, K, w, bias, out, x, D, nxt):
+    res = None
+    if nxt is not None and LN_EPILOGUE and a.dtype == torch.bfloat16:
+        res = ops.linear_fwd_residual_ln(a, M, K, w, bias, out.view(M, D), x.view(M, D), nxt[0], nxt[1])
+    if res is None:
+        ops.linear_fwd(a, M, K, w, bias, out, D, epi=EPI_RESIDUAL, aux=x, ld_aux=D)
+    _ln_next[0] = (weakref.ref(out), nxt[0].data_ptr(), nxt[1].data_ptr(), res) if res is not None else None
+
+
+def _layernorm_in(x, D, M, g, b, adt):
+    ent = _ln_next[0]
+    _ln_next[0] = None
+    if (ent is not None and ent[0]() is x and ent[1] == g.data_ptr() and ent[2] == b.data_ptr() and adt == torch.bfloat16
+            and ent[3][0].shape == (M, D)):
+        return ent[3]
+    return ops.layernorm_fwd(x, D, M, D, g, b, adt)
 
 
 
@@ -459,7 +483,7 @@
 
     @staticmethod
     @_fwd
-    def forward(ctx, x, g, b, wqkv, bqkv, wo, bo, heads, scale, prec):
+    def forward(ctx, x, g, b, wqkv, bqkv, wo, bo, heads, scale, prec, nxt=None):
         adt = ops.act_dtype(prec)
         B, T, D = x.shape
         M = B * T
@@ -469,7 +493,7 @@
         inner = inner3 // 3
         ctx.x6 = adt == torch.float32 and ops.x6_block_ok(M, D, inner3, inner)
         if not (ctx.x6 and D <= 1024):
-            y, mean, rstd = ops.layernorm_fwd(x, D, M, D, g, b, adt)
+            y, mean, rstd = _layernorm_in(x, D, M, g, b, adt)
         if ctx.x6:
             dh = inner // heads
             y6, mean, rstd = ops.layernorm_fwd_split(x, D, M, D, g, b) if D <= 1024 else (ops.split_ex(y, M, D), mean, rstd)
@@ -515,7 +539,7 @@
             o = ops.cast(ops.attention_pv_fp32(probs, q32, B, T, heads, dh), adt)
             lse = None
         out = torch.empty_like(x)
-        ops.linear_fwd(o.view(M, inner), M, inner, wo, bo, out, D, epi=EPI_RESIDUAL, aux=x, ld_aux=D)
+        _residual_out(o.view(M, inner), M, inner, wo, bo, out, x, D, nxt)
         if lse is None and probs is None:
             probs = x.new_empty(0)
         ctx.save_for_backward(x, g, mean, rstd, y, qkv, o, lse if lse is not None else probs, wqkv, wo)
@@ -559,7 +583,7 @@
             dy = torch.empty(M, D, dtype=torch.float32, device=x.device)
             ops.nt_x6(dq6, wqkv, "dx", M, dy)
             dx, dg, db = _ln_bwd_with_side(dy, x, D, g, b, mean, rstd, dout, M, torch.float32, ctx.up_bias)
-            return dx, dg, db, dwqkv, dbqkv, dwo, dbo, None, None, None
+            return dx, dg, db, dwqkv, dbqkv, dwo, dbo, None, None, None, None
         adt = y.dtype
         dout = _c(dout)
         d_act, dbo = _take_side(dout, M, D) if adt == torch.bfloat16 else (None, None)
@@ -585,18 +609,18 @@
         dy = torch.empty(M, D, dtype=adt, device=x.device)
         ops.linear_dx(dqkv.view(M, inner3), M, inner3, wqkv, dy, D)
         dx, dg, db = _ln_bwd_with_side(dy, x, D, g, b, mean, rstd, dout, M, adt, ctx.up_bias)
-        return dx, dg, db, dwqkv, dbqkv, dwo, dbo, None, None, None
-
-
-def attn_block(x, g, b, wqkv, bqkv, wo, bo, heads, scale, prec):
-    return _AttnBlock.apply(x, g, b, wqkv, bqkv, wo, bo, heads, scale, prec)
+        return dx, dg, db, dwqkv, dbqkv, dwo, dbo, None, None, None, None
+
+
+def attn_block(x, g, b, wqkv, bqkv, wo, bo, heads, scale, prec, nxt=None):
+    return _AttnBlock.apply(x, g, b, wqkv, bqkv, wo, bo, heads, scale, prec, nxt)
 
 
 class _MlpBlock(Function):
 
     @staticmethod
     @_fwd
-    def forward(ctx, x, g, b, w1, b1, w2, b2, prec):
+    def forward(ctx, x, g, b, w1, b1, w2, b2, prec, nxt=None):
         adt = ops.act_dtype(prec)
         B, T, D = x.shape
         M = B * T
@@ -605,7 +629,7 @@
         ctx.up_bias = _chain_take(x)
         ctx.x6 = adt == torch.float32 and ops.x6_block_ok(M, D, Hd)
         if not (ctx.x6 and D <= 1024):
-            y, mean, rstd = ops.layernorm_fwd(x, D, M, D, g, b, adt)
+            y, mean, rstd = _layernorm_in(x, D, M, g, b, adt)
         if ctx.x6:
             y6, mean, rstd = ops.layernorm_fwd_split(x, D, M, D, g, b) if D <= 1024 else (ops.split_ex(y, M, D), mean, rstd)
             h = torch.empty(M, Hd, dtype=adt, device=x.device)
@@ -626,7 +650,7 @@
         ops.linear_fwd(y, M, D, w1, b1, a, Hd, epi=(EPI_GELU_GRAD8 if g8 else EPI_GELU_GRAD) if adt == torch.bfloat16 else EPI_GELU,
                        out2=h, ld_out2=Hd)
         out = torch.empty_like(x)
-        ops.linear_fwd(a, M, Hd, w2, b2, out, D, epi=EPI_RESIDUAL, aux=x, ld_aux=D)
+        _residual_out(a, M, Hd, w2, b2, out, x, D, nxt)
         ctx.save_for_backward(x, g, mean, rstd, y, h, a, w1, w2)
         ctx.small = (b, b1, b2)
         _chain_set(out, b2)
@@ -659,7 +683,7 @@
             dy = torch.empty(M, D, dtype=torch.float32, device=x.device)
             ops.nt_x6(dh6, w1, "dx", M, dy)
             dx, dg, db = _ln_bwd_with_side(dy, x, D, g, b, mean, rstd, dout, M, torch.float32, ctx.up_bias)
-            return dx, dg, db, dw1, db1, dw2, db2, None
+            return dx, dg, db, dw1, db1, dw2, db2, None, None
         adt = y.dtype
         dout = _c(dout)
         d_act, db2 = _take_side(dout, M, D) if adt == torch.bfloat16 else (None, None)
@@ -681,11 +705,11 @@
         dy = torch.empty(M, D, dtype=adt, device=x.device)
         ops.linear_dx(dh, M, Hd, w1, dy, D)
         dx, dg, db = _ln_bwd_with_side(dy, x, D, g, b, mean, rstd, dout, M, adt, ctx.up_bias)
-        return dx, dg, db, dw1, db1, dw2, db2, None
-
-
-def mlp_block(x, g, b, w1, b1, w2, b2, prec):
-    return _MlpBlock.apply(x, g, b, w1, b1, w2, b2, prec)
+        return dx, dg, db, dw1, db1, dw2, db2, None, None
+
+
+def mlp_block(x, g, b, w1, b1, w2, b2, prec, nxt=None):
+    return _MlpBlock.apply(x, g, b, w1, b1, w2, b2, prec, nxt)
 
 
 class _ClsHead(Function):
diff --git a/myrtle-vision_amd/myrtle_vision/hip/lib.py b/myrtle-vision_amd/myrtle_vision/hip/lib.py
--- a/myrtle-vision_amd/myrtle_vision/hip/lib.py
+++ b/myrtle-vision_amd/myrtle_vision/hip/lib.py
@@ -8,7 +8,7 @@
 
 MV_F32, MV_BF16, MV_I8, MV_F16 = 0, 1, 2, 3
 EPI_NONE, EPI_GELU, EPI_RESIDUAL, EPI_DGELU, EPI_EMBED, EPI_GELU_GRAD, EPI_MUL, EPI_GELU_Q8 = 0, 1, 2, 3, 4, 5, 6, 7
-EPI_GELU_GRAD8, EPI_MUL8, EPI_SPLIT_DGELU, EPI_SPLIT_GELU = 8, 9, 10, 11
+EPI_GELU_GRAD8, EPI_MUL8, EPI_SPLIT_DGELU, EPI_SPLIT_GELU, EPI_RESIDUAL_LN = 8, 9, 10, 11, 12
 
 _P, _I, _L, _F, _Z = ctypes.c_void_p, ctypes.c_int, ctypes.c_long, ctypes.c_float, ctypes.c_size_t
 _KIND = {"p": _P, "i": _I, "l": _L, "f": _F, "z": _Z, "Q": ctypes.c_uint64}
@@ -24,6 +24,9 @@
     "mv_layernorm_bwd_split": ("pi" "plp" "pp" "ppl" "ppi" "pz" "ii" "pip" "p", _I),
     "mv_gemm_nt_bf16": ("pipipii" "iii" "pi" "pii" "pi" "p", _I),
     "mv_gemm_nt_bf16_scaled": ("pipipii" "iii" "f" "pi" "pii" "pi" "p", _I),
+    "mv_gemm_nt_ln_counters": ("i", _I),
+    "mv_gemm_nt_ln_init": ("pi" "p", _I),
+    "mv_gemm_nt_bf16_ln": ("pipipi" "iii" "p" "pi" "ppfppp" "p" "p", _I),
     "mv_quant_affine_codes": ("pip" "lii" "f" "iiii" "p", _I),
     "mv_quant_float_f16": ("pp" "l" "p", _I),
     "mv_gemm_nt_f16": ("pipipi" "iii" "p" "i" "pi" "pi" "p", _I),
diff --git a/myrtle-vision_amd/myrtle_vision/hip/ops.py b/myrtle-vision_amd/myrtle_vision/hip/ops.py
--- a/myrtle-vision_amd/myrtle_vision/hip/ops.py
+++ b/myrtle-vision_amd/myrtle_vision/hip/ops.py
@@ -7,7 +7,7 @@
 
 from . import lib as _l
 from .lib import (EPI_DGELU, EPI_EMBED, EPI_GELU, EPI_GELU_GRAD, EPI_GELU_GRAD8, EPI_MUL, EPI_MUL8, EPI_NONE, EPI_RESIDUAL,
-                  EPI_SPLIT_DGELU, EPI_SPLIT_GELU, MV_BF16, MV_F32, check,
+                  EPI_RESIDUAL_LN, EPI_SPLIT_DGELU, EPI_SPLIT_GELU, MV_BF16, MV_F32, check,
                   lib)
 
 __all__ = ["EPI_NONE", "EPI_GELU", "EPI_RESIDUAL", "EPI_DGELU", "EPI_EMBED", "EPI_GELU_GRAD", "EPI_MUL", "EPI_GELU_GRAD8", "EPI_MUL8",
@@ -613,6 +613,38 @@
     return out
 
 
+_ln_counters = {}
+MV_ERR_UNSUPPORTED = -4
+
+
+def _ln_epi_counters(M, device):
+    key = (device.index, _s())
+    n = lib().mv_gemm_nt_ln_counters(M)
+    c = _ln_counters.get(key)
+    if c is None or c.numel() < n:
+        c = torch.empty(max(n, 512), dtype=torch.int32, device=device)
+        check(lib().mv_gemm_nt_ln_init(_p(c), c.numel(), _s()), "gemm_nt_ln_init", n=c.numel())
+        _ln_counters[key] = c
+    return c
+
+
+def linear_fwd_residual_ln(x, M, K, weight, bias, out, aux, gamma, beta, eps=1e-5):
+    N = weight.shape[0]
+    pw = prepared_weight(weight)
+    y = torch.empty(M, N, dtype=torch.bfloat16, device=x.device)
+    mean = torch.empty(M, dtype=torch.float32, device=x.device)
+    rstd = torch.empty(M, dtype=torch.float32, device=x.device)
+    t0 = _timer.begin() if _timer is not None else None
+    rc = lib().mv_gemm_nt_bf16_ln(_p(x), K, _p(pw.w), pw.ldw, _p(out), N, M, N, K, _p(bias), _p(aux), N, _p(gamma), _p(beta),
+                                  eps, _p(y), _p(mean), _p(rstd), _p(_ln_epi_counters(M, x.device)), _s())
+    if rc == MV_ERR_UNSUPPORTED:
+        return None
+    check(rc, "gemm_nt_bf16_ln", M=M, N=N, K=K)
+    if t0 is not None:
+        _timer.end("gemm_nt_bf16", t0, 2.0 * M * N * K, shape=f"fwd N{N} K{K} epi{EPI_RESIDUAL_LN}")
+    return y, mean, rstd
+
+
 def linear_dx(dy, M, N, weight, out, ldc, *, ld_dy=None, epi=EPI_NONE, aux=None, ld_aux=0, colsum_partial=None):
     K = weight.shape[1]
     ld_dy = N if ld_dy is None else ld_dy
diff --git a/myrtle-vision_amd/myrtle_vision/models/vit.py b/myrtle-vision_amd/myrtle_vision/models/vit.py
--- a/myrtle-vision_amd/myrtle_vision/models/vit.py
+++ b/myrtle-vision_amd/myrtle_vision/models/vit.py
@@ -75,17 +75,28 @@
             and norm.weight.shape[0] <= 1024 and first.takes_codes(M) and second.takes_codes(M))
 
 
+def _run_block(block, x, after=None):
+    nxt = after.ln_in() if isinstance(block, Residual) and isinstance(after, Residual) else None
+    return block(x) if nxt is None else block(x, ln_next=nxt)
+
+
 class Residual(nn.Module):
     def __init__(self, fn: nn.Module):
         super().__init__()
         self.fn = fn
         self.res_add = FloatFunctional()
 
-    def forward(self, x: torch.Tensor):
-        fused = self._fused(x)
+    def forward(self, x: torch.Tensor, ln_next=None):
+        fused = self._fused(x, ln_next)
         if fused is not None:
             return fused
         return self.res_add.add(self.fn(x), x)
+
+    def ln_in(self):
+        pn = self.fn
+        if type(pn) is PreNorm and _plain(pn.norm, LayerNorm) and self.res_add.plain() and pn.norm.eps == 1e-5:
+            return pn.norm.weight, pn.norm.bias
+        return None
 
     def _fusable_plain(self):
         pn = self.fn
@@ -93,7 +104,7 @@
                 and not self._forward_pre_hooks and not pn._forward_hooks and not pn._forward_pre_hooks
                 and type(pn.fn) is FeedForward and pn.fn.fusable() and not pn.fn._forward_hooks and not pn.fn._forward_pre_hooks)
 
-    def _fused(self, x):
+    def _fused(self, x, ln_next=None):
         pn = self.fn
         if not (type(pn) is PreNorm and _plain(pn.norm, LayerNorm) and self.res_add.plain()):
             return None
@@ -106,10 +117,10 @@
         if type(inner) is Attention and inner.fusable():
             lin_o = inner.to_out[0]
             return F.attn_block(x, pn.norm.weight, pn.norm.bias, inner.to_qkv.weight, inner.to_qkv.bias, lin_o.weight,
-                                lin_o.bias, inner.heads, inner.scale, prec)
+                                lin_o.bias, inner.heads, inner.scale, prec, ln_next)
         if type(inner) is FeedForward and inner.fusable():
             fc1, fc2 = inner.net[0], inner.net[3]
-            return F.mlp_block(x, pn.norm.weight, pn.norm.bias, fc1.weight, fc1.bias, fc2.weight, fc2.bias, prec)
+            return F.mlp_block(x, pn.norm.weight, pn.norm.bias, fc1.weight, fc1.bias, fc2.weight, fc2.bias, prec, ln_next)
         if type(inner) is Attention and inner.int8_pair() is not None:
             fused = inner.int8_fused_forward(x, pn.norm)
             return fused if fused is not None else inner.int8_forward(pn.norm(x), residual=x)
@@ -270,12 +281,13 @@
     def forward(self, x: torch.Tensor):
         last = len(self.layers) - 1
         for i, transformer_block in enumerate(self.layers):
+            prune = i == last and x.dim() == 3 and self._tail_prunable(transformer_block)
             with self.cm_attention:
-                x = transformer_block[0](x)
+                x = _run_block(transformer_block[0], x, None if prune else transformer_block[1])
             with self.cm_feedforward:
-                if i == last and x.dim() == 3 and self._tail_prunable(transformer_block):
+                if prune:
                     x = x[:, :1]
-                x = transformer_block[1](x)
+                x = _run_block(transformer_block[1], x, self.layers[i + 1][0] if i < last else None)
         return x
 
 
```

Result: no change. 7260, median of 6 (-0.2%).
